# fabianschenk/REVO

Measured on AMD Instinct MI355X. Metric: tracked frames/sec at 640x480, 4-level pyramid; ATE vs reference, higher is better.
Workload: dtype f32

## Files before the change

include/revo_hip.h:

```cpp
#ifndef REVO_HIP_H
#define REVO_HIP_H

#include <stddef.h>
#include <stdint.h>

#ifdef __cplusplus
extern "C" {
#endif
#pragma GCC visibility push(default)

#define REVO_MAX_LEVELS 6

enum {
  REVO_OK = 0,
  REVO_ERR_INVALID_ARG = -1,
  REVO_ERR_HIP = -2,
  REVO_ERR_NOT_KEYFRAME = -3,
  REVO_ERR_NOT_ORTHOGONAL = -4,
  REVO_ERR_CAPACITY = -5,
  REVO_ERR_LEVEL = -6,
  REVO_ERR_UNSUPPORTED = -7,
  REVO_ERR_CORRUPT = -8
};

// ... 241 lines not shown
int revo_vo_keyframe(const revo_vo* v, revo_pyr** kf_out, float T_w_kf[16]);

typedef struct revo_vo_multi revo_vo_multi;
typedef struct revo_stream_frame {
  int32_t stream;
  const uint8_t* bgr; size_t bgr_stride;
  const void* depth; size_t depth_stride;
  double timestamp;
} revo_stream_frame;
typedef struct revo_stream_result {
  int32_t stream, new_keyframe;
  double timestamp;
  float pose[16];
} revo_stream_result;
int revo_vo_multi_create(revo_ctx* ctx, int n_streams, int max_queue, revo_vo_multi** out);
void revo_vo_multi_destroy(revo_vo_multi* m);
int revo_vo_multi_submit(revo_vo_multi* m, int n, const revo_stream_frame* frames,
                         int depth_is_u16, double depth_scale_factor);
int revo_vo_multi_step(revo_vo_multi* m, revo_stream_result* out, int* n_out);
int revo_vo_multi_pending(const revo_vo_multi* m, int stream);
int revo_vo_multi_reset(revo_vo_multi* m, int stream);
int revo_vo_multi_num_keyframes(const revo_vo_multi* m, int stream);
int revo_vo_multi_keyframe(const revo_vo_multi* m, int stream, revo_pyr** kf, float T_w_kf[16]);

int revo_vo_multi_submit_device(revo_vo_multi* m, int n, const revo_stream_frame* frames, int depth_is_u16,
                                double depth_scale_factor, void* producer_stream);

typedef struct revo_map revo_map;
int revo_map_create(revo_ctx* ctx, float voxel, int dense, size_t initial_voxels, size_t max_voxels, revo_map** out);
void revo_map_destroy(revo_map* m);
int revo_map_integrate(revo_map* m, const revo_pyr* kf, const float T_w_kf_colmajor[16]);
int revo_map_integrate_many(revo_map* m, int n, const revo_pyr* const* kfs, const float* T_w_kf_colmajor_n16);
int revo_map_clear(revo_map* m);
typedef struct revo_map_info_t {
  size_t voxels;
  size_t points_integrated;
  size_t points_dropped;
  size_t capacity;
  int32_t keyframes;
  int32_t keyframes_rejected;
  int32_t rehashes;
} revo_map_info_t;
int revo_map_info(revo_map* m, revo_map_info_t* out);
int revo_map_extract(revo_map* m, size_t min_count, float* xyz, uint8_t* rgb, uint32_t* count, size_t cap, size_t* n);
int revo_vo_multi_attach_map(revo_vo_multi* mv, int stream, revo_map* m);

typedef struct revo_map_view {
  int32_t width, height;
  float fx, fy, cx, cy, zmin, zmax;
  float T_w_c[16];
  int32_t splat_max;
  uint32_t min_count;
} revo_map_view;
int revo_map_render(revo_map* m, int n, const revo_map_view* views, float* const* depth, uint8_t* const* bgr, uint32_t* covered,
                    int device_out);
int revo_map_render_last_ms(revo_map* m, float* ms);

typedef struct revo_png_info {
  int32_t width, height, bit_depth, color_type, interlace;
  uint64_t idat_bytes;
  uint64_t raw_bytes;
} revo_png_info;
int revo_png_probe(const uint8_t* png, size_t len, revo_png_info* out);

enum { REVO_PNG_BGR8 = 0,
       REVO_PNG_U16 = 1    };
typedef struct revo_png_decoder revo_png_decoder;
int revo_png_decoder_create(revo_ctx* ctx, int max_images, size_t max_compressed_bytes, size_t max_raw_bytes_per_image,
                            revo_png_decoder** out);
void revo_png_decoder_destroy(revo_png_decoder* d);
typedef struct revo_png_job {
  const uint8_t* png; size_t len;
  int32_t format;
  int32_t width, height;
  void* d_dst; size_t dst_stride;
} revo_png_job;
int revo_png_decode_submit(revo_png_decoder* d, int n, const revo_png_job* jobs, void* stream, uint64_t* ticket);
int revo_png_decode_wait(revo_png_decoder* d, uint64_t ticket, int32_t* status);

int revo_debug_census_(int device, unsigned out3[3]);
int revo_debug_gate_timeouts_(int device);
void revo_debug_section_max_(unsigned long long out[12], int reset);
void revo_debug_wait_stats_(unsigned long long out[3]);
int revo_debug_track_profile_(revo_ctx* ctx, float out13[13]);
int revo_debug_batch_profile_(float* out, int n_pairs);

#pragma GCC visibility pop
#ifdef __cplusplus
}
#endif
#endif
```

revo_amd/csrc/revo_dev.h:

```cpp
#pragma once
#include <hip/hip_runtime.h>
#include <stdint.h>
#include "../../include/revo_hip.h"

#define REVO_L REVO_MAX_LEVELS

struct LevelGeom {
  int w, h;
  int npix;
  float fx, fy, cx, cy;
  int patch;
  int hist_w, hist_h;
  int nchunk;
  int chunk_rows;
  int wpr;
  int nms_block_base;
  int has_orig;
  int pix_base;
  int edt_rows;
  int edt_block_base;
  int strip_base;
  int cc_base;
  int band_rows, nbands, band_base;
};
// ... 19 lines not shown
struct FramePlanes {
  uint8_t* gray[REVO_L];
  float* depth[REVO_L];
  uint2* cs[REVO_L];
  uint8_t* edges[REVO_L];
  uint8_t* edges_orig[REVO_L];
  int* scratch[REVO_L];
  float4* pts[REVO_L];
  float4* pts_trk[REVO_L];
  float* dt[REVO_L];
  float4* table[REVO_L];
  uint8_t* hist[REVO_L];
  int* chunk[REVO_L];
  unsigned* cmask[REVO_L];
  uint8_t* vb[REVO_L];
  int* npts;
  int* hist_nz;
  int* strip_tot;
  uint32_t* ebits[REVO_L];
  int* need_full;
  int* hyst_heavy;
  int* tile_base;
  float* stage[REVO_L];
  unsigned short* epre[REVO_L];
  int* stage_base;
};

struct PairDesc {
  const float4* pts[REVO_L];
  const int* npts;
  const float* dt[REVO_L];
  float R[9];
  float T[3];
};

struct TrackParams {
  int pyr_min_lvl, pyr_max_lvl;
  int lvl_begin, lvl_end;
  int check_init;
  int eval_only;
  int kspec[REVO_L];
  int redundant_n;
  float lambda_success_fac, lambda_fail_fac;
  float lambda_initial[REVO_L], step_size_min[REVO_L], convergence_eps[REVO_L];
  int max_its[REVO_L];
  float edge_distance[REVO_L];
  float huber_edge;
  int use_edge_filter;
  struct { float fx, fy, cx, cy; int w, h; } cam[REVO_L];
  int exact_sums;
};

struct EvalOut {
  float A[36];
  float b[6];
  float error;
  float mean_err;
  float sum_w, sum_u;
  int good, bad;
};

#define REVO_MAX_WIDTH 2048
#define NMS_ROWS 6
#define EDT_ROW_PX 1280
#ifndef REVO_HYST_LDS_MAX
#define REVO_HYST_LDS_MAX 158720
#endif
#ifndef TRACK_THREADS
#define TRACK_THREADS 512
#endif
#ifndef TRACK_MAX_CLUSTER
#define TRACK_MAX_CLUSTER 32
#endif
#define TRACK_KMAX 4
#define TRACK_NVAL 48
#define TRACK_NVAL_X 132
#define TRACK_MAIL_NVAL TRACK_NVAL_X

void launch_gray_depth(const PyrGeom& g, const FramePlanes& p, const uint8_t* d_bgr, const float* d_depth_f32,
                       const uint16_t* d_depth_u16, float u16_alpha, int B, hipStream_t s);
void launch_pyrdown(const PyrGeom& g, const FramePlanes& p, int lvl, int B, hipStream_t s, int parts = 3, bool stage_edges = false);
void launch_edge_prefix(const PyrGeom& g, const FramePlanes& p, int B, hipStream_t s);
void launch_canny_nms(const PyrGeom& g, const FramePlanes& p, int B, hipStream_t s);
void launch_hyst(const PyrGeom& g, const FramePlanes& p, int B, hipStream_t s);
void launch_fill(const PyrGeom& g, const FramePlanes& p, int B, hipStream_t s);
void launch_compact(const PyrGeom& g, const FramePlanes& p, int B, hipStream_t s);
void launch_tile_points(const PyrGeom& g, const FramePlanes& p, int B, hipStream_t s, int which = 3);
void launch_pyrdown_bgr(const uint8_t* src, int w, int h, uint8_t* dst, hipStream_t s);
void launch_colored_pcl(const PyrGeom& g, const FramePlanes& p, int frame, int lvl, int dense, const uint8_t* bgr_lvl,
                        int* chunk, unsigned* cmask, int* total, int cap, float* out8, hipStream_t s);
void launch_keyframe(const PyrGeom& g, const FramePlanes& p, int f0, int fstride, int count, hipStream_t s, int which = 3);
int launch_track(const PairDesc* d_descs, const TrackParams& prm, revo_pair_result* d_out, EvalOut* d_eval,
                 int n_pairs, unsigned long long* d_mail, unsigned* epoch_io, int cluster, unsigned* d_resident, hipStream_t s);
void launch_track_gate(unsigned* d_resident, unsigned want, hipStream_t s);
int launch_track_one(const PairDesc& desc, const TrackParams& prm, revo_pair_result* out, EvalOut* eval_out,
                     unsigned long long* d_mail, unsigned* epoch_io, int cluster, unsigned* seq_ptr, unsigned seq_val,
                     unsigned* d_resident, hipStream_t s);
void launch_solve6(const float* d_Ab , int n, float* d_x , hipStream_t s);
int track_blocks_per_cu();
void launch_grad_table(const PyrGeom& g, const FramePlanes& p, int f0, int fstride, int count, hipStream_t s);
struct VoteArgs { float RT[3][12]; const float4* pts[3]; const int* n[3]; };
void launch_vote(const PyrGeom& g, const FramePlanes& curr, int curr_frame, int lvl, int n_clouds, const VoteArgs& va,
                 int* d_marks , int* d_hist8 , unsigned* d_done ,
                 int* h_out8 , unsigned seq_val, int use_orig_edges,
                 hipStream_t s);
void launch_copy_cloud(float4* dst, const float4* src, int* dst_n, const int* src_n, hipStream_t s);
struct VoteDesc {
  float RT[3][12]; const float4* pts[3]; const int* n[3]; int n_clouds;
  const uint8_t* edges; const float* depth;
  int* marks; int* hist8; unsigned* done;
  int* host_out;
};
struct CloudCopyDesc { float4* dst; const float4* src; int* dst_n; const int* src_n; };
struct CopySeg { const void* src; void* dst; size_t bytes; };
void launch_vote_multi(const PyrGeom& g, int lvl, int n, const VoteDesc* d_descs, unsigned seq_val, hipStream_t s);
void launch_copy_cloud_multi(int n, const CloudCopyDesc* d_descs, hipStream_t s);
void launch_copy_segments(int n, const CopySeg* d_segs, hipStream_t s);
```

revo_amd/csrc/revo_host.hip:

```cpp
#include <hip/hip_runtime.h>

#include <cmath>
#include <cstdio>
#include <chrono>
#include <cstring>
#include <atomic>
#include <deque>
#include <mutex>
#include <string>
#include <vector>

#include "revo_dev.h"
#include "revo_internal.h"
#include "revo_mat4.h"
#include "revo_multi.h"
#include "revo_map.h"

static thread_local std::string g_err;
extern "C" const char* revo_last_error(void) { return g_err.c_str(); }
extern "C" const char* revo_version(void) { return "0.1.0 gfx950"; }
extern "C" void revo_set_error_(const char* msg) { g_err = msg ? msg : ""; }

extern "C" void revo_pyr_settings_default(revo_pyr_settings* s) {
  memset(s, 0, sizeof(*s));
  s->width = 640; s->height = 480;
  s->fx = 517.306408f; s->fy = 516.469215f; s->cx = 318.643040f; s->cy = 255.313989f;
  s->pyr_min_lvl = 2; s->pyr_max_lvl = 0;
  s->canny_threshold1 = 150; s->canny_threshold2 = 100;
  s->depth_min = 0.1f; s->depth_max = 5.2f;
  s->use_edge_hist = 1; s->n_percentage = 0.3f;
  s->hist_patch[0] = 20; s->hist_patch[1] = 10; s->hist_patch[2] = 5;
}
extern "C" void revo_opt_settings_default(revo_opt_settings* s) {
  memset(s, 0, sizeof(*s));
  s->lambda_success_fac = 0.5f; s->lambda_fail_fac = 2.0f;
  const float ed[6] = {30, 20, 10, 5, 5, 5};
  for (int i = 0; i < REVO_L; ++i) {
    s->lambda_initial[i] = 0.f; s->step_size_min[i] = 1e-16f; s->convergence_eps[i] = 0.999f;
    s->max_its_per_lvl[i] = 100; s->edge_distance_lvl[i] = ed[i];
  }
  s->huber_edge = 0.3f;
  s->use_edge_filter = 1;
}
extern "C" void revo_tracker_settings_default(revo_tracker_settings* s) {
  s->check_tracking_results = 1; s->check_init_values = 1; s->n_frames_hist_voting = 3;
  s->histogram_level = 2;
}

struct FrameSet {
  int B = 0;
  void* blob = nullptr;
  size_t blob_bytes = 0;
  FramePlanes p{};
  float* own_depth0 = nullptr;
  uint8_t* d_bgr = nullptr;
  float* d_depth = nullptr;
  uint8_t* h_bgr = nullptr;
  float* h_depth = nullptr;
  hipEvent_t ev_ready = nullptr;
  hipStream_t ready_stream = nullptr;
  std::mutex edt_mu;
  std::atomic<bool> edt_pending{false};
  int edt_count = 0;
  hipEvent_t ev_edt = nullptr;
  hipStream_t edt_stream = nullptr;
  bool has_edt = false;
  std::atomic<bool> ref_lists_pending{false};
  hipEvent_t ev_ref = nullptr;
  hipStream_t ref_stream = nullptr;
  bool has_ref = false;
  hipEvent_t ev_free = nullptr;
  hipEvent_t ev_free2 = nullptr;
  hipEvent_t ev_h2d = nullptr;
  bool has_ready = false, has_free = false, has_free2 = false;
};

struct Past {
  float4* d_pts; int* d_n; int n; float T_w[16]; double ts;
  size_t cap;
};

struct Knobs {
  int track_depth;
  int cluster_one;
  int redundant_one;
  int direct_h2d;
  int h2d_max_run_mb;
  bool kspec_one_set;
  int kspec_one[REVO_L];
  int upload_blocks;
  int h2d_kernel;
  int stage_edge_depths;
};

struct revo_ctx {
  std::atomic<int> refs{1};
  int device;
  Knobs knobs;
  revo_pyr_settings ps; revo_opt_settings os; revo_tracker_settings ts;
  PyrGeom geom;
  TrackParams tp;
  hipStream_t stream;
  hipStream_t build_stream;
  std::mutex mu;
  std::vector<FrameSet*> pool;
  int framesets_created = 0;
  std::vector<Past> past_pool;
  PairDesc* h_desc;
  revo_pair_result* h_res;
  EvalOut* h_eval;
  unsigned* h_seq;
  unsigned seq_next = 1;
  unsigned long long* d_mail;
  unsigned mail_epoch = 0;
  int num_cus, blocks_per_cu;
  std::deque<Past> past;
  int* d_marks; int* d_hist8; int* h_hist8; unsigned* d_vote_done;
  std::vector<struct revo_pairs_job*> jobs;
  hipStream_t copy_stream = nullptr, copy_stream2 = nullptr, pair_streams[2] = {nullptr, nullptr};
  hipStream_t vote_stream = nullptr;
  hipEvent_t ev_vote = nullptr;
  hipStream_t frame_copy_stream = nullptr;
  unsigned long long jobs_submitted = 0;
  char* d_pcl = nullptr; float* d_pcl_out; uint8_t* d_pcl_clr[2]; int* d_pcl_chunk; unsigned* d_pcl_mask; int* d_pcl_total;
};

struct revo_pyr {
  revo_ctx* ctx;
  FrameSet* fs;
  int frame;
  bool owns_fs;
  bool is_kf;
  double ts;
  bool table_built;
  bool ref_list_built;
  bool dt_ready = false;
  bool has_colour = false;
};

struct revo_batch {
  revo_ctx* ctx;
  int n_pairs;
  FrameSet* fs;
  std::vector<revo_pyr> views;
  PairDesc* h_descs; PairDesc* d_descs;
  unsigned long long* d_mail;
  unsigned mail_epoch = 0;
  bool identity_uploaded = false;
  int cluster;
  bool defer = true;
  hipStream_t stream;
  hipEvent_t ev0, ev1, ev_upload;
  hipEvent_t ev_trk = nullptr;
// ... 170 lines not shown
  return REVO_OK;
}
extern "C" int revo_debug_gate_timeouts_(int device) {
  TrackChain& ch = g_chain[device & 63];
  std::lock_guard<std::mutex> lk(ch.mu);
  if (!ch.d_resident) return -1;
  unsigned v = 0;
  if (hipMemcpy(&v, ch.d_resident + 1, sizeof(unsigned), hipMemcpyDeviceToHost) != hipSuccess) return -2;
  return (int)v;
}
extern "C" int revo_debug_census_(int device, unsigned out3[3]) {
  TrackChain& ch = g_chain[device & 63];
  std::lock_guard<std::mutex> lk(ch.mu);
  if (!ch.d_resident || !out3) return -1;
  if (hipMemcpy(out3, ch.d_resident, 2 * sizeof(unsigned), hipMemcpyDeviceToHost) != hipSuccess) return -2;
  out3[2] = ch.started_total;
  return 0;
}
static size_t mail_bytes(int n_pairs, int cluster) { return sizeof(unsigned long long) * (size_t)n_pairs * 2 * cluster * TRACK_MAIL_NVAL; }

static size_t align_up(size_t v, size_t a) { return (v + a - 1) / a * a; }

static int frameset_create(revo_ctx* c, int B, bool with_staging, FrameSet** out, bool host_staging = true) {
  const PyrGeom& g = c->geom;
  FrameSet* fs = new FrameSet();
  fs->B = B;
  for (int pass = 0; pass < 2; ++pass) {
    size_t off = 0;
    auto take = [&](size_t bytes) -> void* {
      void* p = pass ? (void*)((char*)fs->blob + off) : nullptr;
      off = align_up(off + bytes, 256);
      return p;
    };
    for (int l = 0; l < g.n_levels; ++l) {
      const LevelGeom& v = g.lv[l];
      const size_t n = (size_t)v.npix * B;
      fs->p.gray[l] = (uint8_t*)take(n);
      fs->p.depth[l] = (float*)take(n * 4);
      fs->p.cs[l] = (uint2*)take((size_t)v.h * v.wpr * 8 * B);
      fs->p.edges[l] = (uint8_t*)take(n);
      fs->p.edges_orig[l] = (uint8_t*)take(n);
      fs->p.scratch[l] = (int*)take(n * 4);
      fs->p.pts[l] = (float4*)take(n * 16);
      fs->p.pts_trk[l] = (float4*)take(n * 16);
      fs->p.dt[l] = (float*)take(n * 4);
      fs->p.table[l] = (float4*)take(n * 16);
      fs->p.hist[l] = (uint8_t*)take((size_t)std::max(1, v.hist_w * v.hist_h) * B);
      fs->p.chunk[l] = (int*)take((size_t)v.w * v.nchunk * B * 4);
      fs->p.cmask[l] = (unsigned*)take((size_t)v.w * v.nchunk * B * 4);
      fs->p.vb[l] = (uint8_t*)take((n + 7) / 8);
      fs->p.ebits[l] = (uint32_t*)take((size_t)v.h * v.wpr * 4 * B);
      if (B > 1 && l < g.n_levels - 1) {
        fs->p.stage[l] = (float*)take(n * 4);
        fs->p.epre[l] = (unsigned short*)take((size_t)v.h * v.wpr * 2 * B);
      }
    }
    fs->own_depth0 = fs->p.depth[0];
    fs->p.npts = (int*)take(sizeof(int) * REVO_L * B);
    fs->p.hist_nz = (int*)take(sizeof(int) * REVO_L * B);
    fs->p.strip_tot = (int*)take(sizeof(int) * (size_t)g.total_strips * B);
    fs->p.tile_base = (int*)take(sizeof(int) * (size_t)g.total_tiles * B);
    fs->p.need_full = (int*)take(sizeof(int) * REVO_L * B);
    fs->p.hyst_heavy = (int*)take(sizeof(int) * B);
    fs->p.stage_base = (int*)take(sizeof(int) * (size_t)g.total_tiles * B);
    if (with_staging) {
      fs->d_bgr = (uint8_t*)take((size_t)g.lv[0].npix * 3 * B);
      fs->d_depth = (float*)take((size_t)g.lv[0].npix * 4 * B);
    }
    if (!pass) {
      fs->blob_bytes = off;
      hipError_t e = hipMalloc(&fs->blob, off);
      if (e != hipSuccess) { delete fs; return fail(REVO_ERR_HIP, std::string("hipMalloc: ") + hipGetErrorString(e)); }
    }
  }
  if (with_staging && host_staging) {
    HIPCHECK(hipHostMalloc((void**)&fs->h_bgr, (size_t)g.lv[0].npix * 3 * B));
    HIPCHECK(hipHostMalloc((void**)&fs->h_depth, (size_t)g.lv[0].npix * 4 * B));
  }
  HIPCHECK(hipEventCreateWithFlags(&fs->ev_ready, hipEventDisableTiming));
  HIPCHECK(hipEventCreateWithFlags(&fs->ev_free, hipEventDisableTiming));
  HIPCHECK(hipEventCreateWithFlags(&fs->ev_free2, hipEventDisableTiming));
  HIPCHECK(hipEventCreateWithFlags(&fs->ev_edt, hipEventDisableTiming));
  HIPCHECK(hipEventCreateWithFlags(&fs->ev_ref, hipEventDisableTiming));
  hipMemsetAsync(fs->p.npts, 0, sizeof(int) * REVO_L * B, c->stream);
  HIPCHECK(hipStreamSynchronize(c->stream));
  *out = fs;
  return REVO_OK;
}
static void frameset_destroy(FrameSet* fs) {
  if (!fs) return;
  if (fs->blob) hipFree(fs->blob);
  if (fs->h_bgr) hipHostFree(fs->h_bgr);
  if (fs->h_depth) hipHostFree(fs->h_depth);
  if (fs->ev_ready) hipEventDestroy(fs->ev_ready);
  if (fs->ev_free) hipEventDestroy(fs->ev_free);
  if (fs->ev_free2) hipEventDestroy(fs->ev_free2);
  if (fs->ev_edt) hipEventDestroy(fs->ev_edt);
  if (fs->ev_ref) hipEventDestroy(fs->ev_ref);
  if (fs->ev_h2d) hipEventDestroy(fs->ev_h2d);
  delete fs;
}

static void enqueue_build(revo_ctx* c, FrameSet* fs, const uint8_t* d_bgr, const float* d_depth_f32,
                          const uint16_t* d_depth_u16, float alpha, hipStream_t s, bool borrow_depth = false,
                          bool with_points = true, int frame0 = 0, int nframes = -1, bool gray_only = false) {
  PyrGeom g = c->geom;
  g.frame0 = frame0;
  const int B = nframes < 0 ? fs->B : nframes;
  fs->p.depth[0] = (borrow_depth && d_depth_f32) ? const_cast<float*>(d_depth_f32) : fs->own_depth0;
  launch_gray_depth(g, fs->p, d_bgr, d_depth_f32, d_depth_u16, alpha, B, s);
  for (int l = 1; l < g.n_levels; ++l) launch_pyrdown(g, fs->p, l, B, s, gray_only ? 1 : 3);
  launch_canny_nms(g, fs->p, B, s);
  launch_hyst(g, fs->p, B, s);
  launch_fill(g, fs->p, B, s);
  if (with_points) launch_tile_points(g, fs->p, B, s);
}

static int enqueue_batch_tail(revo_batch* b, hipStream_t s);
static int batch_wait_tracker(revo_batch* b, hipStream_t s);

static void ctx_free(revo_ctx* c);
extern "C" int revo_ctx_create(int device, const revo_pyr_settings* pyr, const revo_opt_settings* opt,
                               const revo_tracker_settings* trk, revo_ctx** out) {
  if (!pyr || !out) return fail(REVO_ERR_INVALID_ARG, "null argument");
  int ndev = 0;
  if (hipGetDeviceCount(&ndev) != hipSuccess || ndev <= 0)
    return fail(REVO_ERR_HIP, "no HIP device: librevo_hip has no CPU fallback");
  if (device < 0 || device >= ndev) return fail(REVO_ERR_INVALID_ARG, "device ordinal out of range");
  HIPCHECK(hipSetDevice(device));
  revo_ctx* c = new revo_ctx();
  c->device = device;
  c->ps = *pyr;
  c->knobs.track_depth = env_track_depth();
  c->knobs.cluster_one = env_int("REVO_TRACK_CLUSTER_ONE", 0, 0, TRACK_MAX_CLUSTER);
  c->knobs.redundant_one = env_int("REVO_TRACK_REDUNDANT_ONE", 1024, 0, 1 << 30);
  c->knobs.direct_h2d = env_int("REVO_DIRECT_H2D", 1, 0, 1);
  c->knobs.stage_edge_depths = env_int("REVO_STAGE_EDGE_DEPTHS", 0, 0, 1);
  {
    const char* e1 = getenv("REVO_TRACK_KSPEC_ONE");
    const char* eb = getenv("REVO_TRACK_KSPEC");
    const size_t n1 = e1 ? strlen(e1) : 0;
    c->knobs.kspec_one_set = n1 > 0 || !(eb && *eb);
    for (int i = 0; i < REVO_L; ++i) {
      int k = i < 2 ? 3 : TRACK_KMAX;
      if (n1 == 1) k = e1[0] - '0'; else if (n1 > 1) k = e1[std::min<size_t>(i, n1 - 1)] - '0';
      c->knobs.kspec_one[i] = std::max(1, std::min(TRACK_KMAX, k));
    }
  }
  c->knobs.upload_blocks = env_int("REVO_UPLOAD_BLOCKS", 64, 1, 4096);
  c->knobs.h2d_kernel = env_int("REVO_H2D_KERNEL", 0, 0, 1);
  c->knobs.h2d_max_run_mb = env_int("REVO_H2D_MAX_RUN_MB", 64, 1, 4096);
  if (opt) c->os = *opt; else revo_opt_settings_default(&c->os);
  if (trk) c->ts = *trk; else revo_tracker_settings_default(&c->ts);
  std::string why;
  if (build_geom(c->ps, &c->geom, &why)) { delete c; return fail(REVO_ERR_INVALID_ARG, why); }
  build_track_params(c, &c->tp);
  struct Guard { revo_ctx* c; ~Guard() { if (c) ctx_free(c); } } guard{c};
  HIPCHECK(hipStreamCreateWithFlags(&c->stream, hipStreamNonBlocking));
  HIPCHECK(hipStreamCreateWithFlags(&c->build_stream, hipStreamNonBlocking));
  HIPCHECK(hipStreamCreateWithFlags(&c->vote_stream, hipStreamNonBlocking));
  HIPCHECK(hipEventCreateWithFlags(&c->ev_vote, hipEventDisableTiming));
  HIPCHECK(hipHostMalloc((void**)&c->h_desc, sizeof(PairDesc)));
  HIPCHECK(hipHostMalloc((void**)&c->h_res, sizeof(revo_pair_result) * 3));
  HIPCHECK(hipHostMalloc((void**)&c->h_seq, sizeof(unsigned) * 4));
  memset(c->h_seq, 0, sizeof(unsigned) * 4);
  HIPCHECK(hipHostMalloc((void**)&c->h_eval, sizeof(EvalOut)));
  hipDeviceProp_t prop;
  HIPCHECK(hipGetDeviceProperties(&prop, device));
  c->num_cus = prop.multiProcessorCount;
  c->blocks_per_cu = std::min(track_blocks_per_cu(), 2);
  HIPCHECK(hipMalloc((void**)&c->d_mail, mail_bytes(1, TRACK_MAX_CLUSTER)));
  HIPCHECK(hipMemset(c->d_mail, 0, mail_bytes(1, TRACK_MAX_CLUSTER)));
  size_t maxpix = 0;
  for (int l = 0; l < c->geom.n_levels; ++l) maxpix = std::max(maxpix, (size_t)c->geom.lv[l].npix);
  HIPCHECK(hipMalloc((void**)&c->d_marks, sizeof(int) * maxpix));
  HIPCHECK(hipMalloc((void**)&c->d_hist8, sizeof(int) * 8));
  HIPCHECK(hipMalloc((void**)&c->d_vote_done, sizeof(unsigned)));
  HIPCHECK(hipMemset(c->d_marks, 0, sizeof(int) * maxpix));
  HIPCHECK(hipMemset(c->d_hist8, 0, sizeof(int) * 8));
  HIPCHECK(hipMemset(c->d_vote_done, 0, sizeof(unsigned)));
  HIPCHECK(hipHostMalloc((void**)&c->h_hist8, sizeof(int) * 16));
  memset(c->h_hist8, 0, sizeof(int) * 16);
  HIPCHECK(hipDeviceSynchronize());
  guard.c = nullptr;
  *out = c;
  return REVO_OK;
}

static void ctx_free(revo_ctx* c) {
  hipSetDevice(c->device);
  if (c->build_stream) hipStreamSynchronize(c->build_stream);
  if (c->stream) hipStreamSynchronize(c->stream);
  if (c->vote_stream) { (void)hipStreamSynchronize(c->vote_stream); (void)hipStreamDestroy(c->vote_stream); }
  if (c->ev_vote) (void)hipEventDestroy(c->ev_vote);
  for (int k = 0; k < 2; ++k) if (c->pair_streams[k]) (void)hipStreamDestroy(c->pair_streams[k]);
  if (c->copy_stream) (void)hipStreamDestroy(c->copy_stream);
  if (c->copy_stream2) (void)hipStreamDestroy(c->copy_stream2);
// ... 26 lines not shown
      if (c->framesets_created >= total) return REVO_OK;
      c->framesets_created += 1;
    }
    FrameSet* fs = nullptr;
    const int rc = frameset_create(c, 1, true, &fs);
    std::lock_guard<std::mutex> lk(c->mu);
    if (rc) { c->framesets_created -= 1; return rc; }
    c->pool.push_back(fs);
  }
}
extern "C" int revo_ctx_device_(const revo_ctx* c) { return c ? c->device : -1; }
extern "C" void revo_ctx_retain_(revo_ctx* c) { if (c) ctx_ref(c); }
extern "C" void revo_ctx_release_(revo_ctx* c) { if (c) ctx_unref(c); }

extern "C" int revo_ctx_set_tracker(revo_ctx* c, const revo_opt_settings* opt, const revo_tracker_settings* trk) {
  if (!c) return fail(REVO_ERR_INVALID_ARG, "null context");
  std::lock_guard<std::mutex> lk(c->mu);
  if (opt) c->os = *opt;
  if (trk) c->ts = *trk;
  const int exact = c->tp.exact_sums;
  build_track_params(c, &c->tp);
  c->tp.exact_sums = exact;
  while (!c->past.empty()) { c->past_pool.push_back(c->past.front()); c->past.pop_front(); }
  return REVO_OK;
}

extern "C" int revo_ctx_histogram_level(const revo_ctx* c) { return c ? c->ts.histogram_level : -1; }

extern "C" int revo_ctx_set_exact_sums(revo_ctx* c, int on) {
  if (!c) return fail(REVO_ERR_INVALID_ARG, "null context");
  std::lock_guard<std::mutex> lk(c->mu);
  c->tp.exact_sums = on ? 1 : 0;
  return REVO_OK;
}
extern "C" int revo_ctx_exact_sums(const revo_ctx* c) { return c ? c->tp.exact_sums : -1; }

extern "C" int revo_ctx_camera(const revo_ctx* c, int lvl, float out6[6]) {
  if (!c || !out6) return fail(REVO_ERR_INVALID_ARG, "null argument");
  if (lvl < 0 || lvl >= c->geom.n_levels) return fail(REVO_ERR_LEVEL, "level out of range");
  const LevelGeom& v = c->geom.lv[lvl];
  out6[0] = v.fx; out6[1] = v.fy; out6[2] = v.cx; out6[3] = v.cy; out6[4] = (float)v.w; out6[5] = (float)v.h;
  return REVO_OK;
}

static void enqueue_list_side(revo_ctx* c, FrameSet* fs, int f0, int fstride, int count, hipStream_t s) {
  PyrGeom gp = c->geom;
  gp.frame0 = f0; gp.fstride = fstride;
  const bool stage = c->knobs.stage_edge_depths && fs->p.stage[0] != nullptr && c->geom.n_levels > 1;
  if (stage) launch_edge_prefix(gp, fs->p, count, s);
  for (int l = 1; l < c->geom.n_levels; ++l) launch_pyrdown(gp, fs->p, l, count, s, 2, stage);
  gp.pts_staged = stage ? 1 : 0;
  launch_tile_points(gp, fs->p, count, s);
}
static int run_pending_edt(revo_ctx* c, FrameSet* fs, hipStream_t s, bool need_ref_lists = false) {
  std::lock_guard<std::mutex> lk(fs->edt_mu);
  bool behind_build = false;
  if (!fs->edt_pending) {
    if (fs->has_edt && fs->edt_stream != s) HIPCHECK(hipStreamWaitEvent(s, fs->ev_edt, 0));
  } else {
    if (fs->has_ready) HIPCHECK(hipStreamWaitEvent(s, fs->ev_ready, 0));
    behind_build = true;
    enqueue_list_side(c, fs, 1, 2, fs->edt_count, s);
    launch_keyframe(c->geom, fs->p, 0, 2, fs->edt_count, s);
    HIPCHECK(hipGetLastError());
    HIPCHECK(hipEventRecord(fs->ev_edt, s));
    fs->has_edt = true;
    fs->edt_stream = s;
    fs->edt_pending = false;
  }
  if (!need_ref_lists) return REVO_OK;
  if (!fs->ref_lists_pending) {
    if (fs->has_ref && fs->ref_stream != s) HIPCHECK(hipStreamWaitEvent(s, fs->ev_ref, 0));
    return REVO_OK;
  }
  if (!behind_build && fs->has_ready) HIPCHECK(hipStreamWaitEvent(s, fs->ev_ready, 0));
  enqueue_list_side(c, fs, 0, 2, fs->edt_count, s);
  HIPCHECK(hipGetLastError());
  HIPCHECK(hipEventRecord(fs->ev_ref, s));
  fs->has_ref = true;
  fs->ref_stream = s;
  fs->ref_lists_pending = false;
  return REVO_OK;
}
static int wait_edt_before_rebuild(FrameSet* fs, hipStream_t s) {
  std::lock_guard<std::mutex> lk(fs->edt_mu);
  if (fs->has_edt && fs->edt_stream != s) HIPCHECK(hipStreamWaitEvent(s, fs->ev_edt, 0));
  if (fs->has_ref && fs->ref_stream != s) HIPCHECK(hipStreamWaitEvent(s, fs->ev_ref, 0));
  return REVO_OK;
}
typedef unsigned v4u __attribute__((ext_vector_type(4)));
__global__ void __launch_bounds__(256) k_upload_rows(uint8_t* __restrict__ dst, const uint8_t* __restrict__ src, size_t src_stride,
                                                     size_t row_bytes, int rows) {
  const size_t vec = row_bytes / 16, tail0 = vec * 16;
  for (int y = blockIdx.y; y < rows; y += gridDim.y) {
    const uint8_t* s = src + (size_t)y * src_stride;
    uint8_t* d = dst + (size_t)y * row_bytes;
    const bool aligned = (((uintptr_t)s | (uintptr_t)d) & 15) == 0;
    if (aligned) {
      for (size_t i = blockIdx.x * blockDim.x + threadIdx.x; i < vec; i += (size_t)gridDim.x * blockDim.x)
        ((v4u*)d)[i] = __builtin_nontemporal_load((const v4u*)s + i);
      for (size_t i = tail0 + blockIdx.x * blockDim.x + threadIdx.x; i < row_bytes; i += (size_t)gridDim.x * blockDim.x) d[i] = s[i];
    } else {
      for (size_t i = blockIdx.x * blockDim.x + threadIdx.x; i < row_bytes; i += (size_t)gridDim.x * blockDim.x) d[i] = s[i];
    }
  }
}
static hipError_t upload_rows(void* dst, const void* src, size_t src_stride, size_t row_bytes, int rows, int max_blocks, hipStream_t s) {
  void* dsrc = nullptr;
  hipError_t e = hipHostGetDevicePointer(&dsrc, const_cast<void*>(src), 0);
  if (e != hipSuccess) { (void)hipGetLastError(); return e; }
  if (src_stride == row_bytes) {
    const size_t bytes = row_bytes * rows;
    const int blocks = (int)std::min<size_t>((size_t)max_blocks, (bytes / 16 + 255) / 256 + 1);
    hipLaunchKernelGGL(k_upload_rows, dim3(blocks, 1), dim3(256), 0, s, (uint8_t*)dst, (const uint8_t*)dsrc, bytes, bytes, 1);
  } else {
    hipLaunchKernelGGL(k_upload_rows, dim3(2, std::min(rows, 128)), dim3(256), 0, s, (uint8_t*)dst, (const uint8_t*)dsrc, src_stride, row_bytes, rows);
  }
  return hipGetLastError();
}
static std::atomic<unsigned long long> g_sec_max_ns[12];
extern "C" void revo_debug_section_max_(unsigned long long out[12], int reset) {
  for (int i = 0; i < 12; ++i) { out[i] = g_sec_max_ns[i].load(); if (reset) g_sec_max_ns[i].store(0); }
}
extern "C" void revo_debug_section_note_(int i, unsigned long long ns) {
  if (i < 0 || i >= 12) return;
  unsigned long long cur = g_sec_max_ns[i].load(std::memory_order_relaxed);
  while (ns > cur && !g_sec_max_ns[i].compare_exchange_weak(cur, ns)) {}
}
struct SecTimer {
  std::chrono::steady_clock::time_point t = std::chrono::steady_clock::now();
  void lap(int i) {
    const auto n = std::chrono::steady_clock::now();
    revo_debug_section_note_(i, (unsigned long long)std::chrono::duration_cast<std::chrono::nanoseconds>(n - t).count());
    t = n;
  }
};
static int wait_event_polled(hipEvent_t ev) {
  const auto t0 = std::chrono::steady_clock::now();
  for (unsigned spin = 0;; ++spin) {
    const hipError_t e = hipEventQuery(ev);
    if (e == hipSuccess) return REVO_OK;
    if (e != hipErrorNotReady) { (void)hipGetLastError(); return fail(REVO_ERR_HIP, std::string("hipEventQuery: ") + hipGetErrorString(e)); }
    (void)hipGetLastError();
    for (int k = 0; k < 32; ++k) __builtin_ia32_pause();
    if ((spin & 1023) == 1023 && std::chrono::steady_clock::now() - t0 > std::chrono::seconds(2)) break;
  }
  HIPCHECK(hipEventSynchronize(ev));
  return REVO_OK;
}
static int wait_ready_on(revo_ctx* c, const revo_pyr* p, hipStream_t s) {
  if (p->fs->has_ready) HIPCHECK(hipStreamWaitEvent(s, p->fs->ev_ready, 0));
  return run_pending_edt(c, p->fs, s, (p->frame & 1) == 0);
}
static int wait_ready(revo_ctx* c, const revo_pyr* p) { return wait_ready_on(c, p, c->stream); }
static int vote_enqueued(revo_ctx* c, const revo_pyr* p) {
  if (p->owns_fs) return REVO_OK;
  HIPCHECK(hipEventRecord(c->ev_vote, c->vote_stream));
  HIPCHECK(hipStreamWaitEvent(c->stream, c->ev_vote, 0));
  return REVO_OK;
}

static int pyramid_create_common(revo_ctx* c, const uint8_t* bgr, size_t bgr_stride, const void* depth,
                                 size_t depth_stride, bool is_u16, double scale, double ts, revo_pyr** out) {
  if (!c || !bgr || !depth || !out) return fail(REVO_ERR_INVALID_ARG, "null argument");
  HIPCHECK(hipSetDevice(c->device));
  const int w = c->geom.lv[0].w, h = c->geom.lv[0].h;
  if (bgr_stride < (size_t)w * 3 || depth_stride < (size_t)w * (is_u16 ? 2 : 4))
    return fail(REVO_ERR_INVALID_ARG, "stride smaller than a row");
  FrameSet* fs = nullptr;
  SecTimer sec;
  {
    std::lock_guard<std::mutex> lk(c->mu);
    if (!c->pool.empty()) { fs = c->pool.back(); c->pool.pop_back(); }
  }
  sec.lap(0);
  if (!fs) {
    int rc = frameset_create(c, 1, true, &fs);
    if (rc) return rc;
    std::lock_guard<std::mutex> lk(c->mu);
    c->framesets_created += 1;
  }
  const size_t brow = (size_t)w * 3, drow = (size_t)w * (is_u16 ? 2 : 4);
  hipStream_t bs = c->build_stream;
  auto page_locked = [](const void* p) {
    hipPointerAttribute_t at;
    if (hipPointerGetAttributes(&at, p) != hipSuccess) { (void)hipGetLastError(); return false; }
    return at.type == hipMemoryTypeHost;
  };
  const bool direct = c->knobs.direct_h2d && page_locked(bgr) && page_locked(depth) &&
                      page_locked(bgr + (size_t)(h - 1) * bgr_stride + brow - 1) &&
                      page_locked((const char*)depth + (size_t)(h - 1) * depth_stride + drow - 1);
  sec.lap(1);
  if (direct) {
    {
      std::lock_guard<std::mutex> lk(c->mu);
      if (!c->frame_copy_stream) HIPCHECK(hipStreamCreateWithFlags(&c->frame_copy_stream, hipStreamNonBlocking));
    }
    if (!fs->ev_h2d) HIPCHECK(hipEventCreateWithFlags(&fs->ev_h2d, hipEventDisableTiming));
    hipStream_t cs = c->frame_copy_stream;
    if (fs->has_ready) HIPCHECK(hipStreamWaitEvent(cs, fs->ev_ready, 0));
    if (fs->has_free) HIPCHECK(hipStreamWaitEvent(cs, fs->ev_free, 0));
    if (fs->has_free2) HIPCHECK(hipStreamWaitEvent(cs, fs->ev_free2, 0));
    sec.lap(6);
    if (c->knobs.h2d_kernel && upload_rows(fs->d_bgr, bgr, bgr_stride, brow, h, c->knobs.upload_blocks, cs) == hipSuccess) {}
    else if (bgr_stride == brow) HIPCHECK(hipMemcpyAsync(fs->d_bgr, bgr, brow * h, hipMemcpyHostToDevice, cs));
    else HIPCHECK(hipMemcpy2DAsync(fs->d_bgr, brow, bgr, bgr_stride, brow, h, hipMemcpyHostToDevice, cs));
    sec.lap(7);
    if (c->knobs.h2d_kernel && upload_rows(fs->d_depth, depth, depth_stride, drow, h, c->knobs.upload_blocks, cs) == hipSuccess) {}
    else if (depth_stride == drow) HIPCHECK(hipMemcpyAsync(fs->d_depth, depth, drow * h, hipMemcpyHostToDevice, cs));
    else HIPCHECK(hipMemcpy2DAsync(fs->d_depth, drow, depth, depth_stride, drow, h, hipMemcpyHostToDevice, cs));
    sec.lap(8);
    HIPCHECK(hipEventRecord(fs->ev_h2d, cs));
    sec.lap(9);
    HIPCHECK(hipStreamWaitEvent(bs, fs->ev_h2d, 0));
    sec.lap(2);
    { int rc = wait_event_polled(fs->ev_h2d); if (rc) return rc; }
    sec.lap(3);
  } else {
    if (fs->has_ready) HIPCHECK(hipEventSynchronize(fs->ev_ready));
    for (int y = 0; y < h; ++y) memcpy(fs->h_bgr + (size_t)y * brow, bgr + (size_t)y * bgr_stride, brow);
    for (int y = 0; y < h; ++y) memcpy((char*)fs->h_depth + (size_t)y * drow, (const char*)depth + (size_t)y * depth_stride, drow);
    if (fs->has_free) HIPCHECK(hipStreamWaitEvent(bs, fs->ev_free, 0));
    if (fs->has_free2) HIPCHECK(hipStreamWaitEvent(bs, fs->ev_free2, 0));
    HIPCHECK(hipMemcpyAsync(fs->d_bgr, fs->h_bgr, brow * h, hipMemcpyHostToDevice, bs));
    HIPCHECK(hipMemcpyAsync(fs->d_depth, fs->h_depth, drow * h, hipMemcpyHostToDevice, bs));
  }
  const float alpha = is_u16 ? (float)(1.0f / scale) : 0.0f;
  enqueue_build(c, fs, fs->d_bgr, is_u16 ? nullptr : fs->d_depth, is_u16 ? (const uint16_t*)fs->d_depth : nullptr, alpha, bs, true);
  HIPCHECK(hipGetLastError());
  HIPCHECK(hipEventRecord(fs->ev_ready, bs));
  sec.lap(4);
  fs->has_ready = true;
  fs->ready_stream = bs;
  revo_pyr* p = new revo_pyr{c, fs, 0, true, false, ts, false, false};
  ctx_ref(c);
  *out = p;
  return REVO_OK;
}

extern "C" int revo_pyramid_create(revo_ctx* ctx, const uint8_t* bgr, size_t bgr_stride, const float* depth_m,
                                   size_t depth_stride, double timestamp, revo_pyr** out) {
  return pyramid_create_common(ctx, bgr, bgr_stride, depth_m, depth_stride, false, 1.0, timestamp, out);
}
extern "C" int revo_pyramid_create_u16(revo_ctx* ctx, const uint8_t* bgr, size_t bgr_stride, const uint16_t* depth_raw,
                                       size_t depth_stride, double depth_scale_factor, double timestamp, revo_pyr** out) {
  if (!(depth_scale_factor > 0)) return fail(REVO_ERR_INVALID_ARG, "depth_scale_factor must be > 0");
  return pyramid_create_common(ctx, bgr, bgr_stride, depth_raw, depth_stride, true, depth_scale_factor, timestamp, out);
}

extern "C" void revo_pyramid_destroy(revo_pyr* p) {
  if (!p) return;
  if (p->owns_fs) {
    hipSetDevice(p->ctx->device);
    std::lock_guard<std::mutex> lk(p->ctx->mu);
    hipEventRecord(p->fs->ev_free, p->ctx->stream);
    p->fs->has_free = true;
    hipEventRecord(p->fs->ev_free2, p->ctx->vote_stream);
    p->fs->has_free2 = true;
    p->ctx->pool.push_back(p->fs);
  }
  revo_ctx* c = p->owns_fs ? p->ctx : nullptr;
  delete p;
  if (c) ctx_unref(c);
}

extern "C" int revo_pyramid_make_keyframe(revo_pyr* p) {
  if (!p) return fail(REVO_ERR_INVALID_ARG, "null pyramid");
  HIPCHECK(hipSetDevice(p->ctx->device));
  { int rc = wait_ready(p->ctx, p); if (rc) return rc; }
  if (!p->dt_ready) launch_keyframe(p->ctx->geom, p->fs->p, p->frame, 1, 1, p->ctx->stream);
  HIPCHECK(hipGetLastError());
  p->dt_ready = false;
  p->is_kf = true;
  p->table_built = false;
  return REVO_OK;
}
extern "C" int revo_pyramid_prepare_keyframe_(revo_pyr* p) {
  if (!p) return fail(REVO_ERR_INVALID_ARG, "null pyramid");
  if (!p->owns_fs || p->is_kf || p->dt_ready) return REVO_OK;
  HIPCHECK(hipSetDevice(p->ctx->device));
  { int rc = wait_ready(p->ctx, p); if (rc) return rc; }
  launch_keyframe(p->ctx->geom, p->fs->p, p->frame, 1, 1, p->ctx->stream);
  HIPCHECK(hipGetLastError());
  p->dt_ready = true;
  return REVO_OK;
}
extern "C" int revo_pyramid_is_keyframe(const revo_pyr* p) { return p && p->is_kf; }
extern "C" double revo_pyramid_timestamp(const revo_pyr* p) { return p ? p->ts : 0.0; }

extern "C" int revo_pyramid_read(revo_pyr* p, revo_plane what, int lvl, void* dst, size_t cap, size_t* count) {
  if (!p) return fail(REVO_ERR_INVALID_ARG, "null pyramid");
  revo_ctx* c = p->ctx;
  HIPCHECK(hipSetDevice(c->device));
  if (lvl < 0 || lvl >= c->geom.n_levels) return fail(REVO_ERR_LEVEL, "level out of range");
  const LevelGeom& v = c->geom.lv[lvl];
  const FramePlanes& P = p->fs->p;
  const size_t f = (size_t)p->frame;
  { int rc = wait_ready(c, p); if (rc) return rc; }
  HIPCHECK(hipStreamSynchronize(c->stream));
  const void* src = nullptr;
  size_t n = v.npix, esz = 1;
  switch (what) {
    case REVO_PLANE_GRAY: src = P.gray[lvl] + f * v.npix; break;
    case REVO_PLANE_DEPTH: src = P.depth[lvl] + f * v.npix; esz = 4; break;
    case REVO_PLANE_EDGES: src = P.edges[lvl] + f * v.npix; break;
    case REVO_PLANE_EDGES_ORIG:
      src = (v.has_orig ? P.edges_orig[lvl] : P.edges[lvl]) + f * v.npix;
      break;
    case REVO_PLANE_DT:
      if (!p->is_kf) return fail(REVO_ERR_NOT_KEYFRAME, "distance transform not built: call makeKeyframe");
      src = P.dt[lvl] + f * v.npix; esz = 4; break;
    case REVO_PLANE_GRADTABLE:
      if (!p->is_kf) return fail(REVO_ERR_NOT_KEYFRAME, "optimizationStructure not built");
      if (!p->table_built) {
        launch_grad_table(c->geom, P, p->frame, 1, 1, c->stream);
        HIPCHECK(hipGetLastError());
        HIPCHECK(hipStreamSynchronize(c->stream));
        p->table_built = true;
      }
      src = P.table[lvl] + f * v.npix; esz = 16; break;
    case REVO_PLANE_EDGES3D: {
      if (!p->ref_list_built) {
        PyrGeom g1 = c->geom;
        g1.frame0 = p->frame;
        launch_compact(g1, P, 1, c->stream);
        HIPCHECK(hipGetLastError());
        HIPCHECK(hipStreamSynchronize(c->stream));
        p->ref_list_built = true;
      }
      int np = 0;
      HIPCHECK(hipMemcpy(&np, P.npts + f * REVO_L + lvl, sizeof(int), hipMemcpyDeviceToHost));
      n = (size_t)np; src = P.pts[lvl] + f * v.npix; esz = 16; break;
    }
    case REVO_PLANE_EDGES3D_TILED: {
      int np = 0;
      HIPCHECK(hipMemcpy(&np, P.npts + f * REVO_L + lvl, sizeof(int), hipMemcpyDeviceToHost));
      n = (size_t)np; src = P.pts_trk[lvl] + f * v.npix; esz = 16; break;
    }
    case REVO_PLANE_HIST:
      if (v.patch <= 0) { n = 0; src = P.hist[lvl]; break; }
      n = (size_t)v.hist_w * v.hist_h; src = P.hist[lvl] + f * n; break;
    default: return fail(REVO_ERR_INVALID_ARG, "unknown plane");
  }
  if (count) *count = n;
  if (dst) {
    if (n * esz > cap) return fail(REVO_ERR_CAPACITY, "host buffer too small");
    if (n) HIPCHECK(hipMemcpy(dst, src, n * esz, hipMemcpyDeviceToHost));
  }
  return REVO_OK;
}

extern "C" int revo_pyramid_colored_pcl(revo_pyr* p, int lvl, int dense, float* dst8, size_t cap_points, size_t* count) {
  if (!p) return fail(REVO_ERR_INVALID_ARG, "null pyramid");
  revo_ctx* c = p->ctx;
  HIPCHECK(hipSetDevice(c->device));
  if (lvl < 0 || lvl >= c->geom.n_levels) return fail(REVO_ERR_LEVEL, "level out of range");
  if (!(p->owns_fs || p->has_colour) || !p->fs->d_bgr)
    return fail(REVO_ERR_INVALID_ARG, "batch views keep no colour image (rgbFullSize): use revo_pyramid_create");
  { int rc = wait_ready(c, p); if (rc) return rc; }
  std::lock_guard<std::mutex> lk(c->mu);
  const PyrGeom& g = c->geom;
  const size_t n0 = g.lv[0].npix, slots = (size_t)g.lv[0].w * g.lv[0].nchunk;
  if (!c->d_pcl) {
    size_t off = 0;
    auto take = [&](size_t bytes) { size_t o = off; off += (bytes + 255) & ~(size_t)255; return o; };
    const size_t o_out = take(n0 * 32), o_a = take(n0 / 4 * 3 + 3), o_b = take(n0 / 16 * 3 + 3), o_ch = take(slots * 4),
                 o_m = take(slots * 4), o_t = take(4);
    HIPCHECK(hipMalloc((void**)&c->d_pcl, off));
    c->d_pcl_out = (float*)(c->d_pcl + o_out);
    c->d_pcl_clr[0] = (uint8_t*)(c->d_pcl + o_a); c->d_pcl_clr[1] = (uint8_t*)(c->d_pcl + o_b);
    c->d_pcl_chunk = (int*)(c->d_pcl + o_ch); c->d_pcl_mask = (unsigned*)(c->d_pcl + o_m); c->d_pcl_total = (int*)(c->d_pcl + o_t);
  }
  hipStream_t s = c->stream;
  const uint8_t* clr = p->fs->d_bgr + (size_t)p->frame * n0 * 3;
  for (int l = 0; l < lvl; ++l) {
    uint8_t* d = c->d_pcl_clr[l & 1];
    launch_pyrdown_bgr(clr, g.lv[l].w, g.lv[l].h, d, s);
    clr = d;
  }
  const int cap = (int)std::min<size_t>(dst8 ? cap_points : 0, (size_t)g.lv[lvl].npix);
  launch_colored_pcl(g, p->fs->p, p->frame, lvl, dense ? 1 : 0, clr, c->d_pcl_chunk, c->d_pcl_mask, c->d_pcl_total,
                     dst8 ? cap : g.lv[lvl].npix, c->d_pcl_out, s);
  HIPCHECK(hipGetLastError());
  int total = 0;
  HIPCHECK(hipMemcpyAsync(&total, c->d_pcl_total, sizeof(int), hipMemcpyDeviceToHost, s));
  HIPCHECK(hipStreamSynchronize(s));
  if (count) *count = (size_t)total;
  if (dst8) {
    if ((size_t)total > cap_points) return fail(REVO_ERR_CAPACITY, "host buffer too small");
    if (total) HIPCHECK(hipMemcpy(dst8, c->d_pcl_out, (size_t)total * 32, hipMemcpyDeviceToHost));
  }
  return REVO_OK;
}

extern "C" int revo_map_source_(revo_pyr* p, MapSource* out) {
  if (!p || !out) return fail(REVO_ERR_INVALID_ARG, "null pyramid");
  revo_ctx* c = p->ctx;
  HIPCHECK(hipSetDevice(c->device));
  if (!(p->owns_fs || p->has_colour) || !p->fs->d_bgr)
    return fail(REVO_ERR_INVALID_ARG, "batch views keep no colour image (rgbFullSize): use revo_pyramid_create");
  { int rc = wait_ready(c, p); if (rc) return rc; }
  const size_t n0 = c->geom.lv[0].npix, f = (size_t)p->frame;
  out->ctx = c;
  out->depth = p->fs->p.depth[0] + f * n0;
  out->edges = p->fs->p.edges[0] + f * n0;
  out->bgr = p->fs->d_bgr + f * n0 * 3;
  return REVO_OK;
}
extern "C" int revo_map_ctx_geom_(const revo_ctx* c, MapCtxGeom* out) {
  if (!c || !out) return fail(REVO_ERR_INVALID_ARG, "null context");
  const LevelGeom& l = c->geom.lv[0];
  *out = MapCtxGeom{c->device, l.w, l.h, l.fx, l.fy, l.cx, l.cy, c->geom.depth_min, c->geom.depth_max, (void*)c->stream};
  return REVO_OK;
}

static void fill_desc(PairDesc* d, const revo_pyr* ref, const revo_pyr* curr, const float* R, const float* T) {
  const PyrGeom& g = ref->ctx->geom;
  memset(d, 0, sizeof(*d));
  for (int l = 0; l < g.n_levels; ++l) {
    d->pts[l] = curr->fs->p.pts_trk[l] + (size_t)curr->frame * g.lv[l].npix;
    d->dt[l] = ref->fs->p.dt[l] + (size_t)ref->frame * g.lv[l].npix;
  }
  d->npts = curr->fs->p.npts + (size_t)curr->frame * REVO_L;
  if (R) memcpy(d->R, R, sizeof(float) * 9); else { d->R[0] = d->R[4] = d->R[8] = 1.f; }
  if (T) memcpy(d->T, T, sizeof(float) * 3);
}

static int check_pair(const revo_ctx* c, const revo_pyr* ref, const revo_pyr* curr) {
  if (!c || !ref || !curr) return fail(REVO_ERR_INVALID_ARG, "null argument");
  if (ref->ctx != c || curr->ctx != c) return fail(REVO_ERR_INVALID_ARG, "pyramid belongs to another context");
  if (!ref->is_kf) return fail(REVO_ERR_NOT_KEYFRAME, "optimizationStructure not built! (reference frame is not a keyframe)");
  return REVO_OK;
}

static std::atomic<unsigned long long> g_wait_fallbacks{0}, g_wait_max_ns{0}, g_wait_calls{0};
extern "C" void revo_debug_wait_stats_(unsigned long long out[3]) {
  out[0] = g_wait_calls.load(); out[1] = g_wait_fallbacks.load(); out[2] = g_wait_max_ns.load();
}
static int wait_seq(hipStream_t s, volatile unsigned* word, unsigned want) {
  static const int spin_limit = env_int("REVO_WAIT_SPINS", 200000, 1000, 2000000000);
  const auto t0 = std::chrono::steady_clock::now();
  g_wait_calls.fetch_add(1, std::memory_order_relaxed);
  auto note = [&]() {
    const unsigned long long ns = (unsigned long long)std::chrono::duration_cast<std::chrono::nanoseconds>(std::chrono::steady_clock::now() - t0).count();
    unsigned long long cur = g_wait_max_ns.load(std::memory_order_relaxed);
    while (ns > cur && !g_wait_max_ns.compare_exchange_weak(cur, ns)) {}
  };
  for (int spin = 0; spin < spin_limit; ++spin) {
    if (*word == want) { std::atomic_thread_fence(std::memory_order_acquire); note(); return REVO_OK; }
    __builtin_ia32_pause();
  }
  g_wait_fallbacks.fetch_add(1, std::memory_order_relaxed);
  HIPCHECK(hipStreamSynchronize(s));
  note();
  if (*word != want) return fail(REVO_ERR_HIP, "a kernel finished without publishing its result");
  return REVO_OK;
}

static int track_launch(revo_ctx* c, const revo_pyr* ref, const revo_pyr* curr, const float* R, const float* T,
                        const TrackParams& tp, int slot, unsigned* seq_out) {
  fill_desc(c->h_desc, ref, curr, R, T);
  { int rc = wait_ready(c, ref); if (rc) return rc; rc = wait_ready(c, curr); if (rc) return rc; }
  TrackParams tp1 = tp;
  tp1.redundant_n = c->knobs.redundant_one;
  if (c->knobs.kspec_one_set)
    for (int i = 0; i < REVO_L; ++i) tp1.kspec[i] = c->knobs.kspec_one[i];
  const unsigned seq = c->seq_next++;
  if (c->seq_next == 0) c->seq_next = 1;
  const int rc = chained_track_launch(c->device, c->knobs.track_depth, c->stream, [&](unsigned* d_resident) {
    return launch_track_one(*c->h_desc, tp1, c->h_res + slot, c->h_eval, c->d_mail, &c->mail_epoch, pick_cluster(c, 1), c->h_seq + slot,
                            seq, d_resident, c->stream);
  });
  if (rc) return rc;
  *seq_out = seq;
  return REVO_OK;
}
static int track_wait(revo_ctx* c, int slot, unsigned seq) { return wait_seq(c->stream, c->h_seq + slot, seq); }

enum { SINGLE_SLOT = 2 };
static int run_single(revo_ctx* c, const revo_pyr* ref, const revo_pyr* curr, const float* R, const float* T,
                      const TrackParams& tp) {
  unsigned seq = 0;
  int rc = track_launch(c, ref, curr, R, T, tp, SINGLE_SLOT, &seq);
  if (rc) return rc;
// ... 31 lines not shown
  int rc = track_wait(c, slot & 1, seq);
  if (rc) return rc;
  return decode_track(c->h_res[slot & 1], R, T, err, status, nullptr, nullptr);
}

extern "C" int revo_optimizer_track_level(revo_ctx* c, const revo_pyr* ref, const revo_pyr* curr, float R[9], float T[3],
                                          int lvl, revo_residual_info* info, float* err) {
  int rc = check_pair(c, ref, curr);
  if (rc) return rc;
  if (!R || !T) return fail(REVO_ERR_INVALID_ARG, "null pose");
  if (lvl < 0 || lvl >= c->geom.n_levels) return fail(REVO_ERR_LEVEL, "level out of range");
  HIPCHECK(hipSetDevice(c->device));
  std::lock_guard<std::mutex> lk(c->mu);
  TrackParams tp = c->tp;
  tp.lvl_begin = tp.lvl_end = lvl; tp.check_init = 0; tp.eval_only = 0;
  rc = run_single(c, ref, curr, R, T, tp);
  if (rc) return rc;
  return decode_track(c->h_res[SINGLE_SLOT], R, T, err, nullptr, info, nullptr);
}

extern "C" int revo_optimizer_eval(revo_ctx* c, const revo_pyr* ref, const revo_pyr* curr, const float R[9],
                                   const float T[3], int lvl, revo_residual_info* info, float* err, float A[36],
                                   float b[6]) {
  int rc = check_pair(c, ref, curr);
  if (rc) return rc;
  if (!R || !T) return fail(REVO_ERR_INVALID_ARG, "null pose");
  if (lvl < 0 || lvl >= c->geom.n_levels) return fail(REVO_ERR_LEVEL, "level out of range");
  HIPCHECK(hipSetDevice(c->device));
  std::lock_guard<std::mutex> lk(c->mu);
  TrackParams tp = c->tp;
  tp.lvl_begin = tp.lvl_end = lvl; tp.check_init = 0; tp.eval_only = 1;
  rc = run_single(c, ref, curr, R, T, tp);
  if (rc) return rc;
  const EvalOut& e = *c->h_eval;
  if (info) { info->good_pts_edges = e.good; info->bad_pts_edges = e.bad; info->sum_error_unweighted = e.sum_u; info->sum_error_weighted = e.sum_w; }
  if (err) *err = e.mean_err;
  if (A) memcpy(A, e.A, sizeof(float) * 36);
  if (b) memcpy(b, e.b, sizeof(float) * 6);
  return REVO_OK;
}

extern "C" int revo_optimizer_solve6(revo_ctx* c, int n, const float* A36_b6_lambda, float* x6) {
  if (!c || !A36_b6_lambda || !x6 || n <= 0) return fail(REVO_ERR_INVALID_ARG, "bad argument");
  HIPCHECK(hipSetDevice(c->device));
  std::lock_guard<std::mutex> lk(c->mu);
  float *d_in = nullptr, *d_out = nullptr;
  HIPCHECK(hipMalloc((void**)&d_in, sizeof(float) * 43 * (size_t)n));
  hipError_t e = hipMalloc((void**)&d_out, sizeof(float) * 6 * (size_t)n);
  if (e == hipSuccess) e = hipMemcpyAsync(d_in, A36_b6_lambda, sizeof(float) * 43 * (size_t)n, hipMemcpyHostToDevice, c->stream);
  if (e == hipSuccess) { launch_solve6(d_in, n, d_out, c->stream); e = hipGetLastError(); }
  if (e == hipSuccess) e = hipMemcpyAsync(x6, d_out, sizeof(float) * 6 * (size_t)n, hipMemcpyDeviceToHost, c->stream);
  if (e == hipSuccess) e = hipStreamSynchronize(c->stream);
  hipFree(d_in); hipFree(d_out);
  if (e != hipSuccess) return fail(REVO_ERR_HIP, std::string("revo_optimizer_solve6: ") + hipGetErrorString(e));
  return REVO_OK;
}

extern "C" int revo_debug_track_profile_(revo_ctx* c, float out13[13]) {
  if (!c || !out13) return REVO_ERR_INVALID_ARG;
  memcpy(out13, c->h_eval->A, sizeof(float) * 13);
  return REVO_OK;
}

extern "C" int revo_tracker_track_frames(revo_ctx* c, const revo_pyr* ref, const revo_pyr* curr, float R[9], float T[3],
                                         float* err, int* status, revo_residual_info* info, int32_t iters[REVO_MAX_LEVELS]) {
  int rc = check_pair(c, ref, curr);
  if (rc) return rc;
  if (!R || !T) return fail(REVO_ERR_INVALID_ARG, "null pose");
  HIPCHECK(hipSetDevice(c->device));
  std::lock_guard<std::mutex> lk(c->mu);
  TrackParams tp = c->tp;
  tp.eval_only = 0;
  rc = run_single(c, ref, curr, R, T, tp);
  if (rc) return rc;
  return decode_track(c->h_res[SINGLE_SLOT], R, T, err, status, info, iters);
}

static int assess_launch(revo_ctx* c, const float T_w_curr[16], const revo_pyr* curr, int* nframes_out, unsigned* seq_out) {
  *nframes_out = -1;
  if (c->past.empty() || !c->ts.check_tracking_results) return REVO_OK;
  const int hl = c->ts.histogram_level;
  if (hl < 0 || hl >= c->geom.n_levels) return fail(REVO_ERR_LEVEL, "histogram_level outside the pyramid");
  hipStream_t vs = c->vote_stream;
  { int rc = wait_ready_on(c, curr, vs); if (rc) return rc; }
  float inv[16];
  mat4_inverse(T_w_curr, inv);
  int nframes = 0;
  VoteArgs va{};
  for (int fr = 0; fr < c->ts.n_frames_hist_voting && fr < (int)c->past.size() && fr < 3; ++fr) {
    float tf[16];
    mat4_mul(inv, c->past[fr].T_w, tf);
    float* RT = va.RT[fr];
    for (int cc = 0; cc < 3; ++cc) for (int r = 0; r < 3; ++r) RT[cc * 3 + r] = tf[cc * 4 + r];
    RT[9] = tf[12]; RT[10] = tf[13]; RT[11] = tf[14];
    va.pts[fr] = c->past[fr].d_pts;
    va.n[fr] = c->past[fr].d_n;
    ++nframes;
  }
  const int use_orig = c->geom.lv[hl].has_orig;
  const unsigned seq = c->seq_next++;
  if (c->seq_next == 0) c->seq_next = 1;
  launch_vote(c->geom, curr->fs->p, curr->frame, hl, nframes, va, c->d_marks, c->d_hist8, c->d_vote_done, c->h_hist8, seq,
              use_orig, vs);
  HIPCHECK(hipGetLastError());
  { int rc = vote_enqueued(c, curr); if (rc) return rc; }
  *nframes_out = nframes;
  *seq_out = seq;
  return REVO_OK;
}
static int assess_wait(revo_ctx* c, int nframes, unsigned seq, int* status, int32_t hist4[4], int32_t overlaps4[4]) {
  if (status) *status = REVO_TRACKER_STATE_OK;
  if (nframes < 0) return REVO_OK;
  hipStream_t vs = c->vote_stream;
  { int rc = wait_seq(vs, (volatile unsigned*)(c->h_hist8 + 8), seq); if (rc) return rc; }
  const int* hist = c->h_hist8;
  const int* ov = c->h_hist8 + 4;
  const float wts[4] = {0.f, 1.f, 1.25f, 1.5f};
  float overlapMeasure = 0.0f;
  const int hsize = 1 + nframes;
  for (int k = 1; k < hsize; ++k) overlapMeasure += (ov[k] * wts[k]);
  if (hist4) memcpy(hist4, hist, sizeof(int32_t) * 4);
  if (overlaps4) memcpy(overlaps4, ov, sizeof(int32_t) * 4);
  if (status) *status = (overlapMeasure >= ov[0] || hsize < 4) ? REVO_TRACKER_STATE_OK : REVO_TRACKER_STATE_NEW_KF;
  return REVO_OK;
}

extern "C" int revo_tracker_assess_quality(revo_ctx* c, const float T_w_curr[16], const revo_pyr* curr, int* status,
                                           int32_t hist4[4], int32_t overlaps4[4]) {
  if (!c || !T_w_curr || !curr) return fail(REVO_ERR_INVALID_ARG, "null argument");
  if (curr->ctx != c) return fail(REVO_ERR_INVALID_ARG, "pyramid belongs to another context");
  if (hist4) memset(hist4, 0, sizeof(int32_t) * 4);
  if (overlaps4) memset(overlaps4, 0, sizeof(int32_t) * 4);
  if (status) *status = REVO_TRACKER_STATE_OK;
  HIPCHECK(hipSetDevice(c->device));
  std::lock_guard<std::mutex> lk(c->mu);
  int nframes = -1;
  unsigned seq = 0;
  int rc = assess_launch(c, T_w_curr, curr, &nframes, &seq);
  if (rc) return rc;
  return assess_wait(c, nframes, seq, status, hist4, overlaps4);
}
extern "C" int revo_assess_launch_(revo_ctx* c, const float T_w_curr[16], const revo_pyr* curr, int* nframes_out, unsigned* seq_out) {
  if (!c || !T_w_curr || !curr || curr->ctx != c) return fail(REVO_ERR_INVALID_ARG, "bad argument");
  HIPCHECK(hipSetDevice(c->device));
  std::lock_guard<std::mutex> lk(c->mu);
  return assess_launch(c, T_w_curr, curr, nframes_out, seq_out);
}
extern "C" int revo_assess_wait_(revo_ctx* c, int nframes, unsigned seq, int* status, float* ratio_out) {
  if (!c) return fail(REVO_ERR_INVALID_ARG, "null context");
  int32_t ov[4] = {0, 0, 0, 0};
  const int rc = assess_wait(c, nframes, seq, status, nullptr, ov);
  if (ratio_out) {
    *ratio_out = INFINITY;
    if (rc == REVO_OK && nframes >= 3 && ov[0] > 0) {
      const float wts[4] = {0.f, 1.f, 1.25f, 1.5f};
      float m = 0.0f;
      for (int k = 1; k < 1 + nframes && k < 4; ++k) m += ov[k] * wts[k];
      *ratio_out = m / (float)ov[0];
    }
  }
  return rc;
}

static int past_take(revo_ctx* c, size_t need, Past* out) {
  for (size_t k = 0; k < c->past_pool.size(); ++k)
    if (c->past_pool[k].cap >= need) { *out = c->past_pool[k]; c->past_pool.erase(c->past_pool.begin() + k); return REVO_OK; }
  Past p{};
// ... 51 lines not shown
  std::lock_guard<std::mutex> lk(c->mu);
  while ((int)c->past.size() > c->ts.n_frames_hist_voting) {
    c->past_pool.push_back(c->past.front());
    c->past.pop_front();
  }
  return REVO_OK;
}
extern "C" void revo_tracker_reset_past_(revo_ctx* c) {
  if (!c) return;
  std::lock_guard<std::mutex> lk(c->mu);
  while (!c->past.empty()) { c->past_pool.push_back(c->past.front()); c->past.pop_front(); }
}
extern "C" int revo_tracker_past_size(const revo_ctx* c) { return c ? (int)c->past.size() : 0; }

static bool env_defer() {
  return env_int("REVO_EDT_DEFER", 1, 0, 1) && env_int("REVO_DEFER", 2, 0, 3) != 0;
}
extern "C" int revo_batch_create(revo_ctx* c, int n_pairs, revo_batch** out) {
  if (!c || !out || n_pairs <= 0) return fail(REVO_ERR_INVALID_ARG, "bad argument");
  HIPCHECK(hipSetDevice(c->device));
  revo_batch* b = new revo_batch();
  b->ctx = c; b->n_pairs = n_pairs;
  ctx_ref(c);
  int rc = frameset_create(c, 2 * n_pairs, false, &b->fs);
  if (rc) { delete b; ctx_unref(c); return rc; }
  struct Guard { revo_batch* b; ~Guard() { if (b) revo_batch_destroy(b); } } guard{b};
  HIPCHECK(hipStreamCreateWithFlags(&b->stream, hipStreamNonBlocking));
  HIPCHECK(hipEventCreate(&b->ev0)); HIPCHECK(hipEventCreate(&b->ev1));
  HIPCHECK(hipEventCreateWithFlags(&b->ev_upload, hipEventDisableTiming));
  HIPCHECK(hipEventCreateWithFlags(&b->ev_trk, hipEventDisableTiming));
  b->cluster = pick_cluster(c, n_pairs);
  b->defer = env_defer();
  HIPCHECK(hipMalloc((void**)&b->d_mail, mail_bytes(n_pairs, b->cluster)));
  HIPCHECK(hipMemset(b->d_mail, 0, mail_bytes(n_pairs, b->cluster)));
  for (int f = 0; f < 2 * n_pairs; ++f) b->views.push_back(revo_pyr{c, b->fs, f, false, (f % 2) == 0, 0.0, false, false});
  HIPCHECK(hipHostMalloc((void**)&b->h_descs, sizeof(PairDesc) * n_pairs));
  HIPCHECK(hipHostMalloc((void**)&b->h_flags, sizeof(revo_pair_result) * n_pairs));
  HIPCHECK(hipMalloc((void**)&b->d_descs, sizeof(PairDesc) * n_pairs));
  for (int i = 0; i < n_pairs; ++i) fill_desc(&b->h_descs[i], &b->views[2 * i], &b->views[2 * i + 1], nullptr, nullptr);
  HIPCHECK(hipStreamSynchronize(c->stream));
  HIPCHECK(hipStreamSynchronize(nullptr));
  guard.b = nullptr;
  *out = b;
  return REVO_OK;
}
extern "C" void revo_batch_destroy(revo_batch* b) {
  if (!b) return;
  hipSetDevice(b->ctx->device);
  if (b->stream) hipStreamSynchronize(b->stream);
  hipHostFree(b->h_descs); hipHostFree(b->h_flags); hipFree(b->d_descs); hipFree(b->d_mail);
  if (b->ev0) hipEventDestroy(b->ev0);
  if (b->ev1) hipEventDestroy(b->ev1);
  if (b->ev_upload) hipEventDestroy(b->ev_upload);
  if (b->ev_trk) hipEventDestroy(b->ev_trk);
  if (b->stream) hipStreamDestroy(b->stream);
  frameset_destroy(b->fs);
  revo_ctx* c = b->ctx;
  delete b;
  ctx_unref(c);
}

static int batch_wait_tracker(revo_batch* b, hipStream_t s) {
  if (b->has_trk && b->trk_stream != s) HIPCHECK(hipStreamWaitEvent(s, b->ev_trk, 0));
  return REVO_OK;
}
static int batch_wait_build(revo_batch* b, hipStream_t s) {
  if (b->defer) return REVO_OK;
  if (b->fs->has_ready && b->fs->ready_stream != s) HIPCHECK(hipStreamWaitEvent(s, b->fs->ev_ready, 0));
  return REVO_OK;
}
static int batch_mark_tracker(revo_batch* b, hipStream_t s) {
  HIPCHECK(hipEventRecord(b->ev_trk, s));
  b->has_trk = true;
  b->trk_stream = s;
  return REVO_OK;
}

static int enqueue_batch_tail(revo_batch* b, hipStream_t s) {
  const PyrGeom& g = b->ctx->geom;
  if (b->defer) {
    std::lock_guard<std::mutex> lk(b->fs->edt_mu);
    b->fs->edt_pending = true; b->fs->edt_count = b->n_pairs;
    b->fs->ref_lists_pending = true;
  } else {
    launch_tile_points(g, b->fs->p, b->fs->B, s);
    launch_keyframe(g, b->fs->p, 0, 2, b->n_pairs, s);
  }
  return REVO_OK;
}

static int batch_build_f32(revo_batch* b, const uint8_t* d_bgr, const float* d_depth, void* stream, bool borrow) {
  if (!b || !d_bgr || !d_depth) return fail(REVO_ERR_INVALID_ARG, "null argument");
  HIPCHECK(hipSetDevice(b->ctx->device));
  hipStream_t s = stream ? (hipStream_t)stream : b->stream;
  { int rc = wait_edt_before_rebuild(b->fs, s); if (rc) return rc; }
  { int rc = batch_wait_tracker(b, s); if (rc) return rc; }
  enqueue_build(b->ctx, b->fs, d_bgr, d_depth, nullptr, 0.f, s, borrow, false, 0, -1, b->defer);
  { int rc = enqueue_batch_tail(b, s); if (rc) return rc; }
  HIPCHECK(hipGetLastError());
  HIPCHECK(hipEventRecord(b->fs->ev_ready, s));
  b->fs->has_ready = true;
  b->fs->ready_stream = s;
  for (auto& v : b->views) { v.table_built = false; v.ref_list_built = false; }
  return REVO_OK;
}
extern "C" int revo_batch_build(revo_batch* b, const uint8_t* d_bgr, const float* d_depth, void* stream) {
  return batch_build_f32(b, d_bgr, d_depth, stream, false);
}
extern "C" int revo_batch_build_borrow(revo_batch* b, const uint8_t* d_bgr, const float* d_depth, void* stream) {
  return batch_build_f32(b, d_bgr, d_depth, stream, true);
}

static int batch_upload_init(revo_batch* b, const float* h_init_RT, hipStream_t s) {
  if (!h_init_RT && b->identity_uploaded) return REVO_OK;
  b->identity_uploaded = (h_init_RT == nullptr);
  HIPCHECK(hipEventSynchronize(b->ev_upload));
  for (int i = 0; i < b->n_pairs; ++i) {
    PairDesc& d = b->h_descs[i];
    if (h_init_RT) { memcpy(d.R, h_init_RT + 12 * i, sizeof(float) * 9); memcpy(d.T, h_init_RT + 12 * i + 9, sizeof(float) * 3); }
    else { memset(d.R, 0, sizeof(d.R)); d.R[0] = d.R[4] = d.R[8] = 1.f; memset(d.T, 0, sizeof(d.T)); }
  }
  HIPCHECK(hipMemcpyAsync(b->d_descs, b->h_descs, sizeof(PairDesc) * b->n_pairs, hipMemcpyHostToDevice, s));
  HIPCHECK(hipEventRecord(b->ev_upload, s));
  return REVO_OK;
}

extern "C" int revo_batch_prepare(revo_batch* b, void* stream) {
  if (!b) return fail(REVO_ERR_INVALID_ARG, "null argument");
  HIPCHECK(hipSetDevice(b->ctx->device));
  hipStream_t s = stream ? (hipStream_t)stream : b->stream;
  return run_pending_edt(b->ctx, b->fs, s);
}

extern "C" int revo_batch_track_only(revo_batch* b, const float* h_init_RT, revo_pair_result* d_results, void* stream) {
  if (!b || !d_results) return fail(REVO_ERR_INVALID_ARG, "null argument");
  HIPCHECK(hipSetDevice(b->ctx->device));
  hipStream_t s = stream ? (hipStream_t)stream : b->stream;
  { int rc0 = batch_wait_tracker(b, s); if (rc0) return rc0; }
  int rc = batch_upload_init(b, h_init_RT, s);
  if (rc) return rc;
  TrackParams tp = b->ctx->tp;
  tp.eval_only = 0;
  { int rc1 = batch_wait_build(b, s); if (rc1) return rc1; }
  { int rc2 = run_pending_edt(b->ctx, b->fs, s); if (rc2) return rc2; }
  b->last_results = d_results;
  rc = chained_track_launch(b->ctx->device, b->ctx->knobs.track_depth, s, [&](unsigned* d_resident) {
    if (b->tev0) (void)hipEventRecord(b->tev0, s);
    const int n_wg = launch_track(b->d_descs, tp, d_results, nullptr, b->n_pairs, b->d_mail, &b->mail_epoch, b->cluster, d_resident, s);
    if (b->tev1) (void)hipEventRecord(b->tev1, s);
    b->tev0 = b->tev1 = nullptr;
    return n_wg;
  });
  if (rc) return rc;
  return batch_mark_tracker(b, s);
}
extern "C" void revo_batch_time_next_grid_(revo_batch* b, void* ev0, void* ev1) {
  if (b) { b->tev0 = (hipEvent_t)ev0; b->tev1 = (hipEvent_t)ev1; }
}

extern "C" int revo_batch_build_u16(revo_batch* b, const uint8_t* d_bgr, const uint16_t* d_depth_raw,
                                    double depth_scale_factor, void* stream) {
  if (!b || !d_bgr || !d_depth_raw) return fail(REVO_ERR_INVALID_ARG, "null argument");
  if (!(depth_scale_factor > 0.0)) return fail(REVO_ERR_INVALID_ARG, "depth_scale_factor must be positive");
  HIPCHECK(hipSetDevice(b->ctx->device));
  hipStream_t s = stream ? (hipStream_t)stream : b->stream;
  { int rc = wait_edt_before_rebuild(b->fs, s); if (rc) return rc; }
// ... 212 lines not shown
extern "C" int revo_track_pairs(revo_ctx* c, int n, const revo_pair_in* pairs, int depth_is_u16, double depth_scale_factor,
                                revo_pair_out* out) {
  revo_pairs_job* j = nullptr;
  const int rc = revo_track_pairs_submit(c, n, pairs, depth_is_u16, depth_scale_factor, &j);
  if (rc) return rc;
  return revo_track_pairs_wait(j, out);
}

extern "C" int revo_batch_profile_build(revo_batch* b, const uint8_t* d_bgr, const float* d_depth, int reps, revo_stage_times* out) {
  if (!b || !d_bgr || !d_depth || !out || reps <= 0) return fail(REVO_ERR_INVALID_ARG, "bad argument");
  revo_ctx* c = b->ctx;
  HIPCHECK(hipSetDevice(c->device));
  hipStream_t s = b->stream;
  { int rc = wait_edt_before_rebuild(b->fs, s); if (rc) return rc; }
  { int rc = batch_wait_tracker(b, s); if (rc) return rc; }
  memset(out, 0, sizeof(*out));
  PyrGeom g = c->geom;
  g.frame0 = 0;
  FrameSet* fs = b->fs;
  const int B = fs->B, L = g.n_levels;
  fs->p.depth[0] = const_cast<float*>(d_depth);
  struct Stage { const char* name; int a, w; };
  std::vector<Stage> st;
  st.push_back({"k_gray_depth", 0, 0});
  for (int l = 1; l < L; ++l) st.push_back({"k_pyrdown_gray", l, 1});
  st.push_back({"k_canny_nms4", 0, 0});
  st.push_back({"hysteresis", 0, 0});
  st.push_back({"k_fill", 0, 0});
  const bool stage = c->knobs.stage_edge_depths && fs->p.stage[0] != nullptr && L > 1;
  PyrGeom gp = g;
  gp.pts_staged = stage ? 1 : 0;
  if (stage) st.push_back({"k_edge_prefix", 0, 0});
  for (int l = 1; l < L; ++l) st.push_back({"k_pyrdown_depth", l, 2});
  st.push_back({"k_tile_count", 0, 1});
  st.push_back({"k_pts_tiles", 0, 2});
  st.push_back({"k_edt_cols", 0, 1});
  st.push_back({"k_edt_rows", 0, 2});
  const int n = (int)st.size();
  if (n > REVO_MAX_STAGES) return fail(REVO_ERR_CAPACITY, "too many stages");
  struct Events {
    std::vector<hipEvent_t> v;
    ~Events() { for (hipEvent_t e : v) if (e) (void)hipEventDestroy(e); }
  } evs;
  evs.v.assign(n + 1, nullptr);
  std::vector<hipEvent_t>& ev = evs.v;
  for (auto& e : ev) HIPCHECK(hipEventCreate(&e));
  std::vector<double> sum(n, 0.0);
  for (int r = 0; r < reps; ++r) {
    HIPCHECK(hipEventRecord(ev[0], s));
    for (int i = 0; i < n; ++i) {
      const std::string nm = st[i].name;
      if (nm == "k_gray_depth") launch_gray_depth(g, fs->p, d_bgr, d_depth, nullptr, 0.f, B, s);
      else if (nm == "k_pyrdown_gray") launch_pyrdown(g, fs->p, st[i].a, B, s, 1);
      else if (nm == "k_pyrdown_depth") launch_pyrdown(g, fs->p, st[i].a, B, s, 2, stage);
      else if (nm == "k_edge_prefix") launch_edge_prefix(g, fs->p, B, s);
      else if (nm == "k_canny_nms4") launch_canny_nms(g, fs->p, B, s);
      else if (nm == "hysteresis") launch_hyst(g, fs->p, B, s);
      else if (nm == "k_fill") launch_fill(g, fs->p, B, s);
      else if (nm == "k_tile_count" || nm == "k_pts_tiles") launch_tile_points(gp, fs->p, B, s, st[i].w);
      else launch_keyframe(g, fs->p, 0, 2, b->n_pairs, s, st[i].w);
      HIPCHECK(hipGetLastError());
      HIPCHECK(hipEventRecord(ev[i + 1], s));
    }
    HIPCHECK(hipStreamSynchronize(s));
    for (int i = 0; i < n; ++i) {
      float ms = 0.f;
      HIPCHECK(hipEventElapsedTime(&ms, ev[i], ev[i + 1]));
      sum[i] += ms * 1e3;
    }
  }
  out->n = n;
  for (int i = 0; i < n; ++i) {
    out->us[i] = (float)(sum[i] / reps);
    if (std::string(st[i].name).rfind("k_pyrdown", 0) == 0) snprintf(out->name[i], sizeof(out->name[i]), "%s[%d]", st[i].name, st[i].a);
    else snprintf(out->name[i], sizeof(out->name[i]), "%s", st[i].name);
  }
  {
    std::lock_guard<std::mutex> lk(fs->edt_mu);
    fs->edt_pending = false;
    fs->ref_lists_pending = false;
    HIPCHECK(hipEventRecord(fs->ev_edt, s));
    fs->has_edt = true; fs->edt_stream = s;
    fs->has_ref = false;
  }
  HIPCHECK(hipEventRecord(fs->ev_ready, s));
  fs->has_ready = true; fs->ready_stream = s;
  for (auto& v : b->views) { v.table_built = false; v.ref_list_built = false; }
  return REVO_OK;
}

extern "C" int revo_batch_frame(revo_batch* b, int frame, revo_pyr** out) {
  if (!b || !out || frame < 0 || frame >= 2 * b->n_pairs) return fail(REVO_ERR_INVALID_ARG, "bad frame index");
  *out = &b->views[frame];
  return REVO_OK;
}

extern "C" int revo_batch_time_tracker(revo_batch* b, const float* h_init_RT, revo_pair_result* d_results, void* stream,
                                       int reps, float* ms_mean) {
  if (!b || !d_results || !ms_mean || reps <= 0) return fail(REVO_ERR_INVALID_ARG, "bad argument");
  HIPCHECK(hipSetDevice(b->ctx->device));
  hipStream_t s = stream ? (hipStream_t)stream : b->stream;
  { int rc0 = batch_wait_tracker(b, s); if (rc0) return rc0; }
  int rc = batch_upload_init(b, h_init_RT, s);
  if (rc) return rc;
  TrackParams tp = b->ctx->tp;
  tp.eval_only = 0;
  { int rc1 = batch_wait_build(b, s); if (rc1) return rc1; }
  { int rc2 = run_pending_edt(b->ctx, b->fs, s); if (rc2) return rc2; }
  float total = 0.f;
  for (int r = 0; r < reps; ++r) {
    HIPCHECK(hipEventRecord(b->ev0, s));
    rc = chained_track_launch(b->ctx->device, b->ctx->knobs.track_depth, s, [&](unsigned* d_resident) {
      return launch_track(b->d_descs, tp, d_results, nullptr, b->n_pairs, b->d_mail, &b->mail_epoch, b->cluster, d_resident, s);
    });
    if (rc) return rc;
    HIPCHECK(hipEventRecord(b->ev1, s));
    HIPCHECK(hipEventSynchronize(b->ev1));
    float ms = 0.f;
    HIPCHECK(hipEventElapsedTime(&ms, b->ev0, b->ev1));
    total += ms;
  }
  *ms_mean = total / (float)reps;
  return batch_mark_tracker(b, s);
}

struct revo_mdev {
  revo_ctx* c = nullptr;
  int S = 0, cluster = 1, hl = 0;
  TrackParams tp;
  revo_tracker_settings ts;
  FrameSet* kf = nullptr;
  std::vector<revo_pyr> kf_views;
  std::vector<FrameSet*> pool, all;
  PairDesc* h_descs = nullptr; PairDesc* d_descs = nullptr;
  revo_pair_result* d_res = nullptr; revo_pair_result* h_res = nullptr;
  unsigned long long* d_mail = nullptr;
  unsigned mail_epoch = 0;
  VoteDesc* h_vdesc = nullptr; VoteDesc* d_vdesc = nullptr;
  int* d_marks = nullptr; int* d_hist8 = nullptr; unsigned* d_done = nullptr; int* h_vout = nullptr;
  unsigned seq = 0;
  CloudCopyDesc* h_cdesc = nullptr; CloudCopyDesc* d_cdesc = nullptr;
  CopySeg* h_segs = nullptr; CopySeg* d_segs = nullptr; size_t seg_cap = 0;
  std::vector<std::deque<Past>> past;
  std::vector<Past> past_pool;
  size_t cloud_cap = 0;
  hipEvent_t ev_trk = nullptr, ev_vdesc = nullptr, ev_cdesc = nullptr, ev_segs = nullptr, ev_h2d = nullptr, ev_prod = nullptr;
};

extern "C" void revo_mdev_destroy_(revo_mdev* m) {
  if (!m) return;
  revo_ctx* c = m->c;
  hipSetDevice(c->device);
  (void)hipStreamSynchronize(c->stream);
  (void)hipStreamSynchronize(c->build_stream);
  (void)hipStreamSynchronize(c->vote_stream);
  for (FrameSet* fs : m->all) frameset_destroy(fs);
  frameset_destroy(m->kf);
  for (auto& q : m->past) for (auto& p : q) { hipFree(p.d_pts); hipFree(p.d_n); }
  for (auto& p : m->past_pool) { hipFree(p.d_pts); hipFree(p.d_n); }
  hipHostFree(m->h_descs); hipFree(m->d_descs); hipFree(m->d_res); hipHostFree(m->h_res); hipFree(m->d_mail);
  hipHostFree(m->h_vdesc); hipFree(m->d_vdesc); hipFree(m->d_marks); hipFree(m->d_hist8); hipFree(m->d_done); hipHostFree(m->h_vout);
  hipHostFree(m->h_cdesc); hipFree(m->d_cdesc); hipHostFree(m->h_segs); hipFree(m->d_segs);
  for (hipEvent_t e : {m->ev_trk, m->ev_vdesc, m->ev_cdesc, m->ev_segs, m->ev_h2d, m->ev_prod}) if (e) hipEventDestroy(e);
  (void)hipGetLastError();
  delete m;
  ctx_unref(c);
// ... 324 lines not shown
```

revo_amd/csrc/revo_pyramid.hip:

```cpp
#include "revo_dev.h"
#include <type_traits>

namespace {

#ifdef REVO_BUILD_PRIO
#define BUILD_PRIO() __builtin_amdgcn_s_setprio(REVO_BUILD_PRIO)
#else
#define BUILD_PRIO()
#endif

__device__ __forceinline__ int level_of(const PyrGeom& g, int v, int LevelGeom::*base) {
  int l = 0;
#pragma unroll
  for (int k = 1; k < REVO_L; ++k)
    if (k < g.n_levels && v >= g.lv[k].*base) l = k;
  return l;
}
__device__ __forceinline__ int clampi(int v, int lo, int hi) { return v < lo ? lo : (v > hi ? hi : v); }
__device__ __forceinline__ int reflect101(int i, int n) {
  if (i < 0) i = -i;
  if (i >= n) i = 2 * n - 2 - i;
  return i;
}

// ... 238 lines not shown
  const int x = xg * 4;
  const bool active = x < w;
  const uint8_t* gray = pl.gray[l] + (size_t)f * lv.npix;
  const bool has_prev = x > 0, has_next = x + 4 < w;
  const int xo = active ? x : 0;
  const int o_prev = (active && has_prev) ? xo - 4 : xo, o_next = (active && has_next) ? xo + 4 : xo;
  const uint32_t cm_left = (active && has_prev) ? ~0u : 0u, cm_right = (active && has_next) ? ~0u : 0u;
  struct Raw { uint32_t prev, m0, next; };
  auto load_raw = [&](int r) -> Raw {
    const int rr = clampi(r, 0, h - 1);
    const uint8_t* row = gray + (size_t)rr * w;
    Raw q;
    q.m0 = *reinterpret_cast<const uint32_t*>(row + xo);
    q.prev = *reinterpret_cast<const uint32_t*>(row + o_prev);
    q.next = *reinterpret_cast<const uint32_t*>(row + o_next);
    return q;
  };
  auto make_hrow = [&](Raw q) -> HRow4 {
    if (!has_prev) q.prev = (q.m0 & 0xffu) * 0x01010101u;
    if (!has_next) q.next = (q.m0 >> 24) * 0x01010101u;
    return hrow4(q.prev, q.m0, q.next);
  };
  HRow4 H0, H1, H2;
  MRow4 M0, M1, M2;
  DRow4 D0, D1, D2;
  {
    const Raw r0 = load_raw(y0 - 2), r1 = load_raw(y0 - 1), r2 = load_raw(y0), r3 = load_raw(y0 + 1);
    H0 = make_hrow(r0); H1 = make_hrow(r1); H2 = make_hrow(r2);
    mag_row4(H0, H1, H2, cm_left, cm_right, active && y0 - 1 >= 0, M0, D0);
    H0 = make_hrow(r3);
  }
  Raw ahead = load_raw(y0 + 2);
  mag_row4(H1, H2, H0, cm_left, cm_right, active, M1, D1);
  uint2* out = pl.cs[l] + ((size_t)f * h + y0) * lv.wpr + (xg >> 3);
  const int sh = 4 * (threadIdx.x & 7);
  auto emit = [&](int i, uint32_t cb, uint32_t sb) {
    uint32_t cw = cb << sh, sw = sb << sh;
    cw |= (uint32_t)__builtin_amdgcn_update_dpp(0, (int)cw, 0xB1, 0xf, 0xf, true);
    sw |= (uint32_t)__builtin_amdgcn_update_dpp(0, (int)sw, 0xB1, 0xf, 0xf, true);
    cw |= (uint32_t)__builtin_amdgcn_update_dpp(0, (int)cw, 0x4E, 0xf, 0xf, true);
    sw |= (uint32_t)__builtin_amdgcn_update_dpp(0, (int)sw, 0x4E, 0xf, 0xf, true);
    cw |= (uint32_t)__builtin_amdgcn_update_dpp(0, (int)cw, 0x141, 0xf, 0xf, true);
    sw |= (uint32_t)__builtin_amdgcn_update_dpp(0, (int)sw, 0x141, 0xf, 0xf, true);
    if ((threadIdx.x & 7) == 0 && y0 + i < h) out[(size_t)i * lv.wpr] = make_uint2(cw, sw);
  };
#define NMS_STEP4(i, Ha, Hb, Hc, Ma, Mb, Mc, Db, Dc)                                  \
  {                                                                                   \
    Hc = make_hrow(ahead);                                                            \
    if ((i) < NMS_R - 1) ahead = load_raw(y0 + (i) + 3);                              \
    mag_row4(Ha, Hb, Hc, cm_left, cm_right, active && y0 + (i) + 1 < h, Mc, Dc);      \
    uint32_t cb, sb;                                                                  \
    nms_row4(Ma, Mb, Mc, Db, g.canny_low, g.canny_high, &cb, &sb);                    \
    emit((i), cb, sb);                                                                \
  }
  NMS_STEP4(0, H2, H0, H1, M0, M1, M2, D1, D2)
  NMS_STEP4(1, H0, H1, H2, M1, M2, M0, D2, D0)
  NMS_STEP4(2, H1, H2, H0, M2, M0, M1, D0, D1)
  NMS_STEP4(3, H2, H0, H1, M0, M1, M2, D1, D2)
  NMS_STEP4(4, H0, H1, H2, M1, M2, M0, D2, D0)
  NMS_STEP4(5, H1, H2, H0, M2, M0, M1, D0, D1)
#undef NMS_STEP4
}

#ifndef HYST_THREADS
#define HYST_THREADS 1024
#endif
__device__ __forceinline__ uint32_t dil3(uint32_t a, uint32_t al, uint32_t ar) {
  return a | __builtin_amdgcn_alignbit(a, al, 31) | __builtin_amdgcn_alignbit(ar, a, 1);
}
__device__ __forceinline__ uint32_t run_fill(uint32_t C, uint32_t S) {
  const uint32_t up = ((C + S) ^ C) & C;
  const uint32_t rC = __builtin_bitreverse32(C), rS = __builtin_bitreverse32(S);
  const uint32_t dn = __builtin_bitreverse32(((rC + rS) ^ rC) & rC);
  return up | dn | S;
}

#ifdef REVO_HYST_PROFILE
#define HP(i) if (threadIdx.x == 0) hp[i] = clock64()
#define HA(i) if (threadIdx.x == 0) { const long long now_ = clock64(); ha[i] += now_ - hlast; hlast = now_; }
#else
#define HP(i)
#define HA(i)
#endif
template <bool C_IN_LDS, bool E_GLOBAL = false>
__device__ __forceinline__ void hyst_level(const PyrGeom& g, const FramePlanes& pl, const int l, const int f, uint32_t* s_mem) {
  static_assert(!(C_IN_LDS && E_GLOBAL), "the candidate bitmap is in LDS only when the edge bitmap is");
#ifdef REVO_HYST_PROFILE
  long long hp[12], ha[8], hlast = 0;
  for (int i = 0; i < 12; ++i) hp[i] = 0;
  for (int i = 0; i < 8; ++i) ha[i] = 0;
  int dbg_sweeps = 0, dbg_bands = 0;
#endif
  HP(0);
  const LevelGeom& lv = g.lv[l];
  const int w = lv.w, h = lv.h, wpr = lv.wpr;
  const int pitch = wpr;
  const int nwords = h * wpr;
  const int e_words = (h + 2) * pitch + 2;
  uint32_t* Cl = s_mem;
  uint32_t* Ebase = C_IN_LDS ? s_mem + (REVO_HYST_LDS_MAX / 4 - e_words)
                  : (E_GLOBAL ? reinterpret_cast<uint32_t*>(pl.scratch[l] + (size_t)f * g.lv[l].npix) : s_mem);
  uint32_t* E = Ebase + 1;
  const uint2* cs = pl.cs[l] + (size_t)f * h * wpr;
  const int tid = threadIdx.x;
  for (int i = tid; i < pitch + 1; i += HYST_THREADS) { Ebase[i] = 0u; Ebase[e_words - 1 - i] = 0u; }
  for (int i = tid; i < nwords; i += HYST_THREADS) {
    const uint2 v = cs[i];
    E[pitch + i] = v.y;
    if (C_IN_LDS) Cl[i] = v.x & ~v.y;
  }
  __syncthreads();
  HP(1);
  bool done = false;
#ifdef REVO_HYST_PROFILE
  int dbg_runs = -1, dbg_t = 0, dbg_a = 0;
#endif
  if (C_IN_LDS) {
    unsigned short* Bs = reinterpret_cast<unsigned short*>(Cl + nwords);
    uint32_t* parent = Cl + nwords + (nwords + 2) / 2;
    const int table_words = (int)(REVO_HYST_LDS_MAX / 4) - (nwords + (nwords + 2) / 2);
    const int cap = min(table_words / 2, table_words - e_words);
    const int cap_keep = (table_words - e_words) / 2;
    __shared__ int s_wsum[HYST_THREADS / 64];
    __shared__ int s_total, s_promoted;
#ifdef REVO_HYST_PROFILE
    __shared__ int s_dbg[4];
    if (tid < 4) s_dbg[tid] = 0;
#endif
    auto weak = [&](int wi) -> uint32_t { return Cl[wi]; };
    auto starts = [](uint32_t wk) -> uint32_t { return wk & ~(wk << 1); };
    const float inv_wpr = 1.0f / (float)wpr;
    const uint32_t FLAG = 0x80000000u, IDM = 0x7fffffffu;
#ifdef REVO_HYST_PROFILE
    hlast = clock64();
#endif
    for (int sweep = 0; sweep < 64 && !done; ++sweep) {
#ifdef REVO_HYST_PROFILE
      ++dbg_sweeps;
#endif
      {
        const int wpt = (nwords + HYST_THREADS - 1) / HYST_THREADS;
        const int w0 = min(nwords, tid * wpt), w1 = min(nwords, w0 + wpt);
        int mine = 0;
        for (int wi = w0; wi < w1; ++wi) mine += __popc(starts(weak(wi)));
        int incl = mine;
#pragma unroll
        for (int o = 1; o < 64; o <<= 1) {
          const int v = __shfl_up(incl, o);
          if ((tid & 63) >= o) incl += v;
        }
        __syncthreads();
        if ((tid & 63) == 63) s_wsum[tid >> 6] = incl;
        if (tid == 0) s_promoted = 0;
        __syncthreads();
        int before = incl - mine;
        for (int k = 0; k < (tid >> 6); ++k) before += s_wsum[k];
        if (tid == HYST_THREADS - 1) { s_total = before + mine; Bs[nwords] = (unsigned short)min(65535, before + mine); }
        for (int wi = w0; wi < w1; ++wi) {
          Bs[wi] = (unsigned short)before;
          before += __popc(starts(weak(wi)));
        }
        __syncthreads();
      }
      const int nruns = s_total;
      HA(0);
#ifdef REVO_HYST_PROFILE
      if (sweep == 0) dbg_runs = nruns;
// ... 144 lines not shown
    __syncthreads();
  }
  if (!done) {
    __shared__ unsigned short s_list[HYST_THREADS];
    __shared__ unsigned char s_act[2][HYST_THREADS];
    __shared__ int s_n;
  const int max_strips = HYST_THREADS / wpr;
  const int rpt = (h + max_strips - 1) / max_strips;
  const int nstrips = (h + rpt - 1) / rpt;
  const int n_items = nstrips * wpr;
  s_act[0][tid] = 0; s_act[1][tid] = 0;
  if (tid == 0) s_n = 0;
  __syncthreads();
  int n_list = n_items;
#ifndef REVO_HYST_MAXIT
#define REVO_HYST_MAXIT 8192
#endif
  for (int it = 0; it < REVO_HYST_MAXIT; ++it) {
    const int wb = it & 1;
    bool changed = false;
    if (tid < n_list) {
      const int item = it == 0 ? tid : (int)s_list[tid];
      const int strip = item / wpr, c = item - strip * wpr;
      const int r0 = strip * rpt, r1 = min(h, r0 + rpt) - 1;
      uint32_t* Ec = E + pitch + c;
      const uint32_t lm = c > 0 ? ~0u : 0u, rm = c < wpr - 1 ? ~0u : 0u;
      auto Cat = [&](int r) -> uint32_t { return C_IN_LDS ? (Cl[r * wpr + c] | Ec[r * pitch]) : cs[r * wpr + c].x; };
      uint32_t prev_d = dil3(Ec[(r0 - 1) * pitch], Ec[(r0 - 1) * pitch - 1] & lm, Ec[(r0 - 1) * pitch + 1] & rm);
      uint32_t cur = Ec[r0 * pitch], cl = Ec[r0 * pitch - 1] & lm, cr = Ec[r0 * pitch + 1] & rm;
      for (int r = r0; r <= r1; ++r) {
        const uint32_t nx = Ec[(r + 1) * pitch], nl = Ec[(r + 1) * pitch - 1] & lm, nr = Ec[(r + 1) * pitch + 1] & rm;
        const uint32_t Cw = Cat(r);
        const uint32_t hz = __builtin_amdgcn_alignbit(cur, cl, 31) | __builtin_amdgcn_alignbit(cr, cur, 1);
        const uint32_t F = run_fill(Cw, cur | (Cw & (prev_d | dil3(nx, nl, nr) | hz)));
        if (F != cur) { Ec[r * pitch] = F; changed = true; }
        prev_d = dil3(F, cl, cr);
        cur = nx; cl = nl; cr = nr;
      }
      prev_d = dil3(cur, cl, cr);
      cur = Ec[r1 * pitch]; cl = Ec[r1 * pitch - 1] & lm; cr = Ec[r1 * pitch + 1] & rm;
      for (int r = r1; r >= r0; --r) {
        const uint32_t nx = Ec[(r - 1) * pitch], nl = Ec[(r - 1) * pitch - 1] & lm, nr = Ec[(r - 1) * pitch + 1] & rm;
        const uint32_t Cw = Cat(r);
        const uint32_t hz = __builtin_amdgcn_alignbit(cur, cl, 31) | __builtin_amdgcn_alignbit(cr, cur, 1);
        const uint32_t F = run_fill(Cw, cur | (Cw & (prev_d | dil3(nx, nl, nr) | hz)));
        if (F != cur) { Ec[r * pitch] = F; changed = true; }
        prev_d = dil3(F, cl, cr);
        cur = nx; cl = nl; cr = nr;
      }
      if (changed) s_act[wb][item] = 1;
    }
    if (!__syncthreads_or(changed ? 1 : 0)) break;
    bool act = false;
    if (tid < n_items) {
      const int strip = tid / wpr, c = tid - strip * wpr;
      const unsigned char* a = s_act[wb];
#pragma unroll
      for (int ds = -1; ds <= 1; ++ds)
#pragma unroll
        for (int dc = -1; dc <= 1; ++dc) {
          const int ss = strip + ds, cc = c + dc;
          if (ss >= 0 && ss < nstrips && cc >= 0 && cc < wpr) act = act || a[ss * wpr + cc] != 0;
        }
    }
    const unsigned long long m = __ballot(act);
    int base = 0;
    if ((tid & 63) == 0 && m) base = atomicAdd(&s_n, __popcll(m));
    base = __shfl(base, 0);
    if (act) s_list[base + __popcll(m & ((1ull << (tid & 63)) - 1ull))] = (unsigned short)tid;
    s_act[wb ^ 1][tid] = 0;
    __syncthreads();
    n_list = s_n;
    __syncthreads();
    if (tid == 0) s_n = 0;
  }
  __syncthreads();
  }
  __syncthreads();
  HP(5);
  uint8_t* edges = pl.edges[l] + (size_t)f * lv.npix;
  uint8_t* orig = lv.has_orig ? pl.edges_orig[l] + (size_t)f * lv.npix : nullptr;
  const bool rows16 = (w & 15) == 0;
  const float inv_w = 1.0f / (float)w;
  for (int i = tid; i < lv.npix / 16; i += HYST_THREADS) {
    const int p = i * 16;
    int y = (int)(((float)p + 0.5f) * inv_w);
    y += (y + 1) * w <= p ? 1 : (y * w > p ? -1 : 0);
    const int x = p - y * w;
    uint32_t o[4];
    if (rows16) {
      const uint32_t bits = (E[(y + 1) * pitch + (x >> 5)] >> (x & 31)) & 0xffffu;
#pragma unroll
      for (int q = 0; q < 4; ++q) o[q] = ((((bits >> (4 * q)) & 0xfu) * 0x00204081u) & 0x01010101u) * 0xffu;
    } else {
#pragma unroll
      for (int q = 0; q < 4; ++q) {
        int xx = x + 4 * q, yy = y;
        while (xx >= w) { xx -= w; yy += 1; }
        const uint32_t bits = (E[(yy + 1) * pitch + (xx >> 5)] >> (xx & 31)) & 0xfu;
        o[q] = ((bits * 0x00204081u) & 0x01010101u) * 0xffu;
      }
    }
    const uint4 v = make_uint4(o[0], o[1], o[2], o[3]);
    *reinterpret_cast<uint4*>(edges + p) = v;
    if (orig) *reinterpret_cast<uint4*>(orig + p) = v;
  }
  {
    uint2* csw = pl.cs[l] + (size_t)f * h * wpr;
    for (int i = tid; i < nwords; i += HYST_THREADS) csw[i].y = E[pitch + i];
  }
  HP(6);
  if (lv.patch > 0) {
    const int ntiles = lv.hist_w * lv.hist_h;
    int nz = 0;
    const float inv_hw = 1.0f / (float)lv.hist_w;
    for (int t0 = 0; t0 < ntiles; t0 += HYST_THREADS) {
      const int t = t0 + tid;
      if (t < ntiles) {
        int ty = (int)(((float)t + 0.5f) * inv_hw);
        ty += (ty + 1) * lv.hist_w <= t ? 1 : (ty * lv.hist_w > t ? -1 : 0);
        const int tx = t - ty * lv.hist_w;
        const int xa = tx * lv.patch, xb = xa + lv.patch;
        const int wa = xa >> 5, wb = (xb - 1) >> 5;
        const uint32_t ma = ~0u << (xa & 31), mb = (xb & 31) ? ~0u >> (32 - (xb & 31)) : ~0u;
        const uint32_t m0 = wa == wb ? ma & mb : ma, m1 = wb > wa + 1 ? ~0u : (wb > wa ? mb : 0u), m2 = wb > wa + 1 ? mb : 0u;
        const int o1 = wb > wa ? 1 : 0, o2 = wb > wa + 1 ? 2 : 0;
        const uint32_t* row = E + (ty * lv.patch + 1) * pitch + wa;
        int cnt = 0;
        for (int y = 0; y < lv.patch; ++y, row += pitch) cnt += __popc(row[0] & m0) + __popc(row[o1] & m1) + __popc(row[o2] & m2);
        const uint8_t v = (uint8_t)(cnt & 255);
        pl.hist[l][(size_t)f * ntiles + t] = v;
        nz += v != 0;
      }
    }
    __shared__ int s_nz;
    if (tid == 0) s_nz = 0;
    __syncthreads();
    if (nz) atomicAdd(&s_nz, nz);
    __syncthreads();
    if (tid == 0) pl.hist_nz[f * REVO_L + l] = s_nz;
  }
#ifdef REVO_HYST_PROFILE
  HP(7);
  if (threadIdx.x == 0 && l == 0 && f < 64)
    printf("hyst f=%d: load %lld uf_total %lld [scan %lld record %lld link %lld compress %lld flag %lld resolve %lld] runs %d sweeps %d bands %d uf %d rebuild %lld out %lld hist %lld touched %d atomics %d\n", f,
           hp[1] - hp[0], hp[5] - hp[1], ha[0], ha[1], ha[2], ha[3], ha[4], ha[5], dbg_runs, dbg_sweeps, dbg_bands, (int)done, ha[6], hp[6] - hp[5], hp[7] - hp[6], dbg_t, dbg_a);
#endif
}
template <bool C_IN_LDS, bool E_GLOBAL = false>
__global__ void __launch_bounds__(HYST_THREADS) k_hyst(PyrGeom g, FramePlanes pl, int only_flagged, int n_frames) {
  BUILD_PRIO();
  extern __shared__ uint32_t s_mem[];
  const int n_items = g.n_levels * n_frames;
  if (only_flagged) {
    __shared__ int s_any;
    if (threadIdx.x == 0) s_any = 0;
    __syncthreads();
    for (int item = threadIdx.x; item < n_items; item += HYST_THREADS)
      if (pl.need_full[(g.frame0 + item % n_frames) * REVO_L + item / n_frames]) s_any = 1;
    __syncthreads();
    if (!s_any) return;
  }
  for (int item = blockIdx.x; item < n_items; item += gridDim.x) {
    const int l = item / n_frames;
    const int f = g.frame0 + item % n_frames;
    if (only_flagged && !pl.need_full[f * REVO_L + l]) continue;
    hyst_level<C_IN_LDS, E_GLOBAL>(g, pl, l, f, s_mem);
    __syncthreads();
  }
}

#ifndef HB_THREADS
#define HB_THREADS 1024
#endif
#ifndef HB_LDS_WORDS
#define HB_LDS_WORDS 16384
#endif
struct BandRef { int l, R0, R1; };
__device__ __forceinline__ BandRef band_ref(const PyrGeom& g, int bi) {
  int l = 0;
#pragma unroll
  for (int k = 1; k < REVO_L; ++k)
    if (k < g.n_levels && bi >= g.lv[k].band_base) l = k;
  const LevelGeom& lv = g.lv[l];
  const int b = bi - lv.band_base;
  BandRef r;
  r.l = l; r.R0 = b * lv.band_rows; r.R1 = min(lv.h, r.R0 + lv.band_rows);
  return r;
}
__device__ __forceinline__ int band_capb(const LevelGeom& lv) {
  const int hb = lv.band_rows, nwb = hb * lv.wpr;
  const int table_words = HB_LDS_WORDS - (nwb + (nwb + 2) / 2);
  const int e_words = (hb + 2) * lv.wpr + 2;
  int cap = min(table_words / 2, table_words - e_words);
  cap = min(cap, 65535);
  const int h_last = lv.h - (lv.nbands - 1) * lv.band_rows;
  cap = min(cap, ((h_last * lv.w - 4 - 2 * lv.wpr) / 8) * 5);
  return max(cap, 0) & ~31;
}
struct BandRec { int* hdr; int* bs_first; int* bs_last; uint32_t* flags; unsigned short* root; uint32_t* rec; };
__device__ __forceinline__ BandRec band_rec(const FramePlanes& pl, const LevelGeom& lv, int l, int f, int R0, int capb) {
  int* base = pl.scratch[l] + (size_t)f * lv.npix + (size_t)R0 * lv.w;
  BandRec r;
  r.hdr = base; r.bs_first = base + 4; r.bs_last = base + 4 + lv.wpr;
  r.flags = reinterpret_cast<uint32_t*>(base + 4 + 2 * lv.wpr);
  r.root = reinterpret_cast<unsigned short*>(base + 4 + 2 * lv.wpr + capb / 32);
  r.rec = reinterpret_cast<uint32_t*>(base + 4 + 2 * lv.wpr + capb / 32 + capb / 2);
  return r;
}

__device__ __forceinline__ void hyst_band(const PyrGeom& g, const FramePlanes& pl, const BandRef br, const int f, uint32_t* s_mem) {
  __shared__ int s_wsum[HB_THREADS / 64];
  __shared__ int s_total;
  const int l = br.l;
  const LevelGeom& lv = g.lv[l];
  const int h = lv.h, wpr = lv.wpr, pitch = wpr;
  const int hb = br.R1 - br.R0, nwb = hb * wpr, e_words = (hb + 2) * pitch + 2;
  const int tid = threadIdx.x;
  uint32_t* Cl = s_mem;
  uint32_t* Ebase = s_mem + (HB_LDS_WORDS - e_words);
  uint32_t* E = Ebase + 1;
  const uint2* cs = pl.cs[l] + ((size_t)f * h + br.R0) * wpr;
  const int capb = band_capb(lv);
  const BandRec rec_out = band_rec(pl, lv, l, f, br.R0, capb);
  auto load_e = [&](bool with_cl) {
    if (tid == 0) { Ebase[0] = 0u; Ebase[e_words - 1] = 0u; }
    for (int c = tid; c < wpr; c += HB_THREADS) {
      E[c] = br.R0 > 0 ? cs[c - wpr].y : 0u;
      E[(hb + 1) * pitch + c] = br.R1 < h ? cs[nwb + c].y : 0u;
    }
    for (int i0 = tid; i0 < nwb; i0 += 4 * HB_THREADS) {
      uint2 v[4];
#pragma unroll
      for (int k = 0; k < 4; ++k) v[k] = cs[min(i0 + k * HB_THREADS, nwb - 1)];
#pragma unroll
      for (int k = 0; k < 4; ++k) {
        const int i = i0 + k * HB_THREADS;
        if (i < nwb) {
          if (with_cl) { E[pitch + i] = v[k].y; Cl[i] = v[k].x & ~v[k].y; }
          else E[pitch + i] = v[k].y | (v[k].x & ~Cl[i]);
        }
      }
    }
  };
  load_e(true);
  __syncthreads();
  unsigned short* Bs = reinterpret_cast<unsigned short*>(Cl + nwb);
  uint32_t* parent = Cl + nwb + (nwb + 2) / 2;
  const int table_words = HB_LDS_WORDS - (nwb + (nwb + 2) / 2);
  const int cap_keep = (table_words - e_words) / 2;
// ... 82 lines not shown
    }
    __syncthreads();
    for (int me = tid; me < nr; me += HB_THREADS) {
      parent[me] = key_of(find(me));
      rec_out.rec[me] = rec[me];
    }
    __syncthreads();
    if (nr > cap_keep) {
      load_e(false);
      __syncthreads();
    }
    for (int wi = tid; wi < nwb; wi += HB_THREADS) {
      const uint32_t wk = Cl[wi];
      if (!wk) continue;
      int r = (int)(((float)wi + 0.5f) * inv_wpr);
      r += (r + 1) * wpr <= wi ? 1 : (r * wpr > wi ? -1 : 0);
      const int c = wi - r * wpr;
      const uint32_t lm = c > 0 ? ~0u : 0u, rm = c < wpr - 1 ? ~0u : 0u;
      const uint32_t* Xc = E + pitch + wi;
      const uint32_t sd = dil3(Xc[-pitch], Xc[-pitch - 1] & lm, Xc[-pitch + 1] & rm) | dil3(Xc[pitch], Xc[pitch - 1] & lm, Xc[pitch + 1] & rm) |
                          __builtin_amdgcn_alignbit(Xc[0], Xc[-1] & lm, 31) | __builtin_amdgcn_alignbit(Xc[1] & rm, Xc[0], 1);
      if (!(wk & sd)) continue;
      const uint32_t touched = run_fill(wk, wk & sd);
      int me = (int)Bs[wi];
      for (uint32_t m = starts(wk); m; m &= m - 1, ++me)
        if (touched & m & (0u - m)) {
          uint32_t* root = &parent[parent[me] & 0xffffu];
          if (!(*root & FLAG)) atomicOr(root, FLAG);
        }
    }
    __syncthreads();
    for (int wi = tid; wi < nwb; wi += HB_THREADS) {
      const uint32_t wk = Cl[wi];
      if (!wk) continue;
      int me = (int)Bs[wi];
      uint32_t prom = 0;
      for (uint32_t m = starts(wk); m; m &= m - 1, ++me)
        if (parent[parent[me] & 0xffffu] & FLAG) prom |= m & (0u - m);
      if (prom) E[pitch + wi] |= run_fill(wk, prom);
    }
    __syncthreads();
  }
  uint32_t* eb = pl.ebits[l] + ((size_t)f * h + br.R0) * wpr;
  for (int i = tid; i < nwb; i += HB_THREADS) eb[i] = E[pitch + i];
  if (tid == 0) { rec_out.hdr[0] = nr; rec_out.hdr[1] = 0; rec_out.hdr[2] = 1; }
  for (int c = tid; c < wpr; c += HB_THREADS) { rec_out.bs_first[c] = Bs[c]; rec_out.bs_last[c] = Bs[(hb - 1) * wpr + c]; }
  for (int i = tid; i < (nr + 31) / 32; i += HB_THREADS) {
    uint32_t bits = 0;
    for (int k = 0; k < 32; ++k) {
      const int me = 32 * i + k;
      if (me < nr && (int)(parent[me] & 0xffffu) == me && (parent[me] & FLAG)) bits |= 1u << k;
    }
    rec_out.flags[i] = bits;
  }
  for (int me = tid; me < nr; me += HB_THREADS) rec_out.root[me] = (unsigned short)(parent[me] & 0xffffu);
}
__global__ void __launch_bounds__(HB_THREADS) k_hyst_band(PyrGeom g, FramePlanes pl) {
  extern __shared__ uint32_t s_mem[];
  const int nB = gridDim.x / g.total_bands;
  hyst_band(g, pl, band_ref(g, blockIdx.x / nB), g.frame0 + blockIdx.x % nB, s_mem);
}

__device__ __forceinline__ bool hyst_frame_is_heavy(const PyrGeom& g, const FramePlanes& pl, int f) {
  __shared__ int s_cnt[HYST_THREADS / 64];
  const LevelGeom& lv = g.lv[0];
  const int nwords = lv.h * lv.wpr;
  const uint2* cs = pl.cs[0] + (size_t)f * nwords;
  int mine = 0;
  for (int i = threadIdx.x; i < nwords; i += HYST_THREADS) {
    const uint2 v = cs[i];
    const uint32_t wk = v.x & ~v.y;
    mine += __popc(wk & ~(wk << 1));
  }
#pragma unroll
  for (int o = 32; o >= 1; o >>= 1) mine += __shfl_xor(mine, o);
  __syncthreads();
  if ((threadIdx.x & 63) == 0) s_cnt[threadIdx.x >> 6] = mine;
  __syncthreads();
  int total = 0;
#pragma unroll
  for (int k = 0; k < HYST_THREADS / 64; ++k) total += s_cnt[k];
  return total >= g.hyst_heavy_runs;
}
__global__ void __launch_bounds__(HYST_THREADS) k_hyst_mixed(PyrGeom g, FramePlanes pl, int n_frames) {
  static_assert(HB_THREADS == HYST_THREADS, "one workgroup shape for both paths");
  extern __shared__ uint32_t s_mem[];
  const int nb0 = g.lv[0].nbands;
  const int n_band_wg = nb0 * n_frames;
  if ((int)blockIdx.x < n_band_wg) {
    const int f = g.frame0 + blockIdx.x % n_frames;
    if (!hyst_frame_is_heavy(g, pl, f)) return;
    hyst_band(g, pl, band_ref(g, blockIdx.x / n_frames), f, s_mem);
    return;
  }
  const int item = blockIdx.x - n_band_wg;
  const int l = item / n_frames, f = g.frame0 + item % n_frames;
  if (l == 0) {
    const bool heavy = hyst_frame_is_heavy(g, pl, f);
    if (threadIdx.x == 0) pl.hyst_heavy[f] = heavy ? 1 : 0;
    if (heavy) return;
  }
  hyst_level<true>(g, pl, l, f, s_mem);
}

#define HS_THREADS 256
#define HS_MAX_BANDS 32
#define HS_MAX_PAIRS 6144
__global__ void __launch_bounds__(HS_THREADS) k_hyst_seam(PyrGeom g, FramePlanes pl, int mixed) {
  extern __shared__ uint32_t s_fl[];
  __shared__ uint2 s_pair[HS_MAX_PAIRS];
  __shared__ int s_npairs;
  __shared__ int s_changed_band[HS_MAX_BANDS];
  const int nB = mixed ? gridDim.x : gridDim.x / g.n_levels;
  const int l = blockIdx.x / nB;
  const int f = g.frame0 + blockIdx.x % nB;
  const LevelGeom& lv = g.lv[l];
  const int nb = lv.nbands;
  if (nb <= 1 || pl.need_full[f * REVO_L + l]) return;
  if (mixed && !pl.hyst_heavy[f]) return;
  const int wpr = lv.wpr, h = lv.h;
  const int tid = threadIdx.x;
  const int capb = band_capb(lv), fw = capb / 32;
  const uint2* cs = pl.cs[l] + (size_t)f * h * wpr;
  for (int b = 0; b < nb; ++b) {
    const BandRec rb = band_rec(pl, lv, l, f, b * lv.band_rows, capb);
    const int n = (rb.hdr[0] + 31) / 32;
    for (int i = tid; i < fw; i += HS_THREADS) s_fl[b * fw + i] = i < n ? rb.flags[i] : 0u;
  }
  if (tid < HS_MAX_BANDS) s_changed_band[tid] = 0;
  if (tid == 0) s_npairs = 0;
  __syncthreads();
  auto starts = [](uint32_t wk) -> uint32_t { return wk & ~(wk << 1); };
  auto weak_at = [&](int y, int c) -> uint32_t { if (c < 0 || c >= wpr) return 0u; const uint2 v = cs[(size_t)y * wpr + c]; return v.x & ~v.y; };
  for (int item = tid; item < (nb - 1) * wpr; item += HS_THREADS) {
    const int sm = item / wpr, c = item - sm * wpr;
    const int yb = (sm + 1) * lv.band_rows, ya = yb - 1;
    const uint32_t Wa = weak_at(ya, c);
    const uint32_t Wl = weak_at(yb, c - 1), Wm = weak_at(yb, c), Wr = weak_at(yb, c + 1);
    if (!Wa || !(Wm | (Wl >> 31) | (Wr & 1u))) continue;
    const BandRec ra = band_rec(pl, lv, l, f, sm * lv.band_rows, capb);
    const BandRec rbb = band_rec(pl, lv, l, f, yb, capb);
    int ida = ra.bs_last[c];
    const int idm = rbb.bs_first[c], idl = c > 0 ? rbb.bs_first[c - 1] : 0, idr = c < wpr - 1 ? rbb.bs_first[c + 1] : 0;
    for (uint32_t m = starts(Wa); m; m &= m - 1, ++ida) {
      const int bit = __ffs(m) - 1;
      const uint32_t t2 = ~(Wa >> bit);
      const int len = t2 ? __ffs(t2) - 1 : 32 - bit;
      const uint32_t ma = (0xffffffffu >> (32 - len)) << bit;
      int roota = -1;
      for (int side = 0; side < 3; ++side) {
        int idb0; uint32_t Wb, hits;
        if (side == 0) { Wb = Wm; hits = Wm & (ma | (ma << 1) | (ma >> 1)); idb0 = idm; }
        else if (side == 1) { Wb = Wl; hits = (ma & 1u) ? (Wl & 0x80000000u) : 0u; idb0 = idl; }
        else { Wb = Wr; hits = (ma >> 31) ? (Wr & 1u) : 0u; idb0 = idr; }
        while (hits) {
          const int hb2 = __ffs(hits) - 1;
          const uint32_t upto = (2u << hb2) - 1u;
          const int k = __popc(starts(Wb) & upto) - 1;
          const uint32_t gap = ~Wb & upto;
          const int first = gap ? 32 - __clz(gap) : 0;
          const uint32_t t3 = ~(Wb >> first);
          const int lenb = t3 ? __ffs(t3) - 1 : 32 - first;
          hits &= ~((0xffffffffu >> (32 - lenb)) << first);
          if (roota < 0) roota = ra.root[ida];
          const int rootb = rbb.root[idb0 + k];
          const int slot = atomicAdd(&s_npairs, 1);
          if (slot < HS_MAX_PAIRS) s_pair[slot] = make_uint2((uint32_t)sm, (uint32_t)roota | ((uint32_t)rootb << 16));
        }
      }
    }
  }
  __syncthreads();
  const int np = s_npairs;
  if (np > HS_MAX_PAIRS) {
    if (tid == 0) pl.need_full[f * REVO_L + l] = 1;
    return;
  }
  for (int it = 0; it < 65536; ++it) {
    bool changed = false;
    for (int i = tid; i < np; i += HS_THREADS) {
      const uint2 pr = s_pair[i];
      const int sm = (int)pr.x, roota = (int)(pr.y & 0xffffu), rootb = (int)(pr.y >> 16);
      uint32_t* fa = s_fl + sm * fw;
      uint32_t* fb = s_fl + (sm + 1) * fw;
      const bool A = (fa[roota >> 5] >> (roota & 31)) & 1u, Bf = (fb[rootb >> 5] >> (rootb & 31)) & 1u;
      if (A != Bf) {
        if (!A) { atomicOr(&fa[roota >> 5], 1u << (roota & 31)); s_changed_band[sm] = 1; }
        else { atomicOr(&fb[rootb >> 5], 1u << (rootb & 31)); s_changed_band[sm + 1] = 1; }
        changed = true;
      }
    }
    if (!__syncthreads_or(changed ? 1 : 0)) break;
  }
  __syncthreads();
  for (int b = 0; b < nb; ++b) {
    if (!s_changed_band[b]) continue;
    const BandRec rb = band_rec(pl, lv, l, f, b * lv.band_rows, capb);
    const int n = (rb.hdr[0] + 31) / 32;
    for (int i = tid; i < n; i += HS_THREADS) rb.flags[i] = s_fl[b * fw + i];
    if (tid == 0) rb.hdr[1] = 1;
  }
}

#define HO_THREADS 512
__global__ void __launch_bounds__(HO_THREADS) k_hyst_out(PyrGeom g, FramePlanes pl, int mixed) {
  extern __shared__ uint32_t s_mem[];
  const int nB = gridDim.x / (mixed ? g.lv[0].nbands : g.total_bands);
  const BandRef br = band_ref(g, blockIdx.x / nB);
  const int f = g.frame0 + blockIdx.x % nB;
  const int l = br.l;
  if (pl.need_full[f * REVO_L + l]) return;
  if (mixed && !pl.hyst_heavy[f]) return;
  const LevelGeom& lv = g.lv[l];
  const int w = lv.w, h = lv.h, wpr = lv.wpr, pitch = wpr;
  const int hb = br.R1 - br.R0, nwb = hb * wpr;
  const int tid = threadIdx.x;
  uint32_t* E = s_mem;
  uint32_t* eb = pl.ebits[l] + ((size_t)f * h + br.R0) * wpr;
  for (int i = tid; i < nwb; i += HO_THREADS) E[i] = eb[i];
  const BandRec rb = band_rec(pl, lv, l, f, br.R0, band_capb(lv));
  const bool promote = rb.hdr[1] != 0;
  __syncthreads();
  if (promote) {
    const int nr = rb.hdr[0];
    for (int me = tid; me < nr; me += HO_THREADS) {
      const int root = rb.root[me];
      if ((rb.flags[root >> 5] >> (root & 31)) & 1u) {
        const uint32_t rc = rb.rec[me];
        atomicOr(&E[rc >> 10], (0xffffffffu >> (31u - (rc & 31u))) << ((rc >> 5) & 31u));
      }
    }
    __syncthreads();
  }
  uint8_t* edges = pl.edges[l] + (size_t)f * lv.npix + (size_t)br.R0 * w;
  uint8_t* orig = lv.has_orig ? pl.edges_orig[l] + (size_t)f * lv.npix + (size_t)br.R0 * w : nullptr;
  const bool rows16 = (w & 15) == 0;
  const float inv_w = 1.0f / (float)w;
  for (int i = tid; i < hb * w / 16; i += HO_THREADS) {
    const int p = i * 16;
    int y = (int)(((float)p + 0.5f) * inv_w);
    y += (y + 1) * w <= p ? 1 : (y * w > p ? -1 : 0);
    const int x = p - y * w;
    uint32_t o[4];
    if (rows16) {
      const uint32_t bits = (E[y * pitch + (x >> 5)] >> (x & 31)) & 0xffffu;
#pragma unroll
      for (int q = 0; q < 4; ++q) o[q] = ((((bits >> (4 * q)) & 0xfu) * 0x00204081u) & 0x01010101u) * 0xffu;
    } else {
#pragma unroll
      for (int q = 0; q < 4; ++q) {
        int xx = x + 4 * q, yy = y;
        while (xx >= w) { xx -= w; yy += 1; }
        const uint32_t bits = (E[yy * pitch + (xx >> 5)] >> (xx & 31)) & 0xfu;
        o[q] = ((bits * 0x00204081u) & 0x01010101u) * 0xffu;
      }
    }
    const uint4 v = make_uint4(o[0], o[1], o[2], o[3]);
    *reinterpret_cast<uint4*>(edges + p) = v;
    if (orig) *reinterpret_cast<uint4*>(orig + p) = v;
  }
  {
    uint2* csw = pl.cs[l] + ((size_t)f * h + br.R0) * wpr;
    for (int i = tid; i < nwb; i += HO_THREADS) csw[i].y = E[i];
  }
  if (lv.patch > 0) {
    const int ty0 = br.R0 / lv.patch, ty1 = min(lv.hist_h, br.R1 / lv.patch);
    const int ntiles = max(0, ty1 - ty0) * lv.hist_w;
    int nz = 0;
    for (int t = tid; t < ntiles; t += HO_THREADS) {
      const int ty = ty0 + t / lv.hist_w, tx = t % lv.hist_w;
      const int xa = tx * lv.patch, xb = xa + lv.patch;
      const int wa = xa >> 5, wb = (xb - 1) >> 5;
      const uint32_t ma = ~0u << (xa & 31), mb = (xb & 31) ? ~0u >> (32 - (xb & 31)) : ~0u;
      const uint32_t m0 = wa == wb ? ma & mb : ma, m1 = wb > wa + 1 ? ~0u : (wb > wa ? mb : 0u), m2 = wb > wa + 1 ? mb : 0u;
      const int o1 = wb > wa ? 1 : 0, o2 = wb > wa + 1 ? 2 : 0;
      const uint32_t* row = E + (ty * lv.patch - br.R0) * pitch + wa;
      int cnt = 0;
      for (int y = 0; y < lv.patch; ++y, row += pitch) cnt += __popc(row[0] & m0) + __popc(row[o1] & m1) + __popc(row[o2] & m2);
      const uint8_t v = (uint8_t)(cnt & 255);
      pl.hist[l][(size_t)f * lv.hist_w * lv.hist_h + (size_t)ty * lv.hist_w + tx] = v;
      nz += v != 0;
    }
#pragma unroll
    for (int o = 32; o > 0; o >>= 1) nz += __shfl_xor(nz, o);
    if ((tid & 63) == 0 && nz) atomicAdd(&pl.hist_nz[f * REVO_L + l], nz);
  }
}

__global__ void __launch_bounds__(1024) k_fill(PyrGeom g, FramePlanes pl, int only_level) {
  BUILD_PRIO();
  const int f = g.frame0 + blockIdx.z;
  const int la = only_level ? only_level : 1, lb = only_level ? only_level + 1 : g.n_levels;
  for (int l = la; l < lb; ++l) {
    const LevelGeom lv = g.lv[l], lf = g.lv[l - 1];
    if (!(g.use_edge_hist && lv.patch > 0 && lf.patch > 0)) continue;
    const float frac = (float)pl.hist_nz[f * REVO_L + l] / (float)(lv.hist_w * lv.hist_h);
    if (frac < g.n_percentage) {
      const uint8_t* top = pl.edges[l - 1] + (size_t)f * lf.npix;
      uint8_t* mod = pl.edges[l] + (size_t)f * lv.npix;
      const uint8_t* hist = pl.hist[l] + (size_t)f * lv.hist_w * lv.hist_h;
      const double thr = g.fill_thr[l];
      const int cw = lf.w / 2, ch = lf.h / 2;
      for (int i = blockIdx.x * 1024 + threadIdx.x; i < cw * ch; i += gridDim.x * 1024) {
        const int y = i / cw, x = i % cw;
        const int yy = 2 * y + 1, xx = 2 * x + 1;
        const int ty = yy / lf.patch, tx = xx / lf.patch;
        if (ty >= lv.hist_h || tx >= lv.hist_w) continue;
        if ((double)hist[(size_t)ty * lv.hist_w + tx] < thr && top[(size_t)yy * lf.w + xx] > 0) {
          mod[(size_t)y * lv.w + x] = 255;
          atomicOr(&(pl.cs[l] + (size_t)f * lv.h * lv.wpr)[(size_t)y * lv.wpr + (x >> 5)].y, 1u << (x & 31));
        }
      }
    }
    __syncthreads();
  }
}

__device__ __forceinline__ uint32_t tile_transpose32(uint32_t v, int r) {
#pragma unroll
  for (int k = 16; k >= 1; k >>= 1) {
    const uint32_t mk = k == 16 ? 0x0000ffffu : k == 8 ? 0x00ff00ffu : k == 4 ? 0x0f0f0f0fu : k == 2 ? 0x33333333u : 0x55555555u;
    const uint32_t t = (uint32_t)__shfl_xor((int)v, k);
    v = (r & k) ? ((v & ~mk) | ((t >> k) & mk)) : ((v & mk) | ((t & mk) << k));
  }
  return v;
}

__device__ __forceinline__ bool depth_ok(float Z, float dmin, float dmax) {
  return isfinite(Z) && Z > dmin && Z < dmax;
}

#define CW_COLS 64
#define CW_LANES 16
#ifndef CW_LANES_COUNT
#define CW_LANES_COUNT 8
#endif
#define CW_MAXCHUNK 64
#define CW_STAGE 4096
template <bool WRITE>
__global__ void __launch_bounds__(CW_COLS * (WRITE ? CW_LANES : CW_LANES_COUNT)) k_compact_walk(PyrGeom g, FramePlanes pl) {
  constexpr int LANES = WRITE ? CW_LANES : CW_LANES_COUNT;
  __shared__ int s_cnt[CW_COLS * CW_MAXCHUNK];
  __shared__ unsigned s_mask[CW_COLS * CW_MAXCHUNK];
  __shared__ float4 s_pts[WRITE ? CW_STAGE : 1];
  const int nB = gridDim.x / g.total_strips;
  const int sx = blockIdx.x / nB;
  const int f = g.frame0 + blockIdx.x % nB;
  const int l = level_of(g, sx, &LevelGeom::strip_base);
  const LevelGeom& lv = g.lv[l];
  const int strip = sx - lv.strip_base;
  const int tid = threadIdx.x, xl = tid & (CW_COLS - 1), cl = tid / CW_COLS;
  const int x = strip * CW_COLS + xl;
  const int ncols = min(CW_COLS, lv.w - strip * CW_COLS);
  const int nslots = ncols * lv.nchunk;
  const size_t slot0 = (size_t)f * lv.w * lv.nchunk + (size_t)strip * CW_COLS * lv.nchunk;
  const float* depth = pl.depth[l] + (size_t)f * lv.npix;
  if (!WRITE) {
    const uint8_t* edges = pl.edges[l] + (size_t)f * lv.npix;
    const bool bit_tiles = l < g.n_levels - 1 && (lv.w & 31) == 0 && lv.chunk_rows == 32;
    if (bit_tiles) {
      const uint2* csw = pl.cs[l] + (size_t)f * lv.h * lv.wpr;
      const uint32_t* vw = reinterpret_cast<const uint32_t*>(pl.vb[l] + (size_t)f * (lv.npix >> 3));
      const int lane = tid & 63, r = lane & 31;
      const int wc = strip * (CW_COLS / 32) + (lane >> 5);
      for (int c = cl; c < lv.nchunk; c += LANES) {
        const int y = c * 32 + r;
        uint32_t v = 0;
        if (y < lv.h && wc < lv.wpr) v = csw[(size_t)y * lv.wpr + wc].y & vw[(size_t)y * lv.wpr + wc];
        v = tile_transpose32(v, r);
        if (x < lv.w) {
          s_mask[xl * lv.nchunk + c] = v;
          s_cnt[xl * lv.nchunk + c] = __popc(v);
        }
      }
    } else
    if (x < lv.w) {
      for (int c = cl; c < lv.nchunk; c += LANES) {
        const int yb = c * lv.chunk_rows, ye = min(lv.h, yb + lv.chunk_rows);
        unsigned em = 0;
#pragma unroll 8
        for (int y = yb; y < ye; ++y) em |= (edges[(size_t)y * lv.w + x] ? 1u : 0u) << (y - yb);
        unsigned vm = 0;
        if (l < g.n_levels - 1) {
          const uint8_t* vb = pl.vb[l] + (size_t)f * (lv.npix >> 3);
          const int vpitch = lv.w >> 3;
          if (em) {
#pragma unroll 8
            for (int y = yb; y < ye; ++y) vm |= ((unsigned)(vb[(size_t)y * vpitch + (x >> 3)] >> (x & 7)) & 1u) << (y - yb);
            vm &= em;
          }
        } else
        for (unsigned m = em; m;) {
          int b[4];
          float Z[4];
#pragma unroll
          for (int j = 0; j < 4; ++j) {
            b[j] = m ? __ffs(m) - 1 : -1;
            m &= m - 1;
// ... 348 lines not shown
  const int i = blockIdx.x * 256 + threadIdx.x;
  if (i >= dw * dh) return;
  const int x = i % dw, y = i / dw;
  const int kk[5] = {1, 4, 6, 4, 1};
  int acc[3] = {0, 0, 0};
#pragma unroll
  for (int j = 0; j < 5; ++j) {
    const uint8_t* row = src + (size_t)reflect101(2 * y + j - 2, h) * w * 3;
    int rs[3] = {0, 0, 0};
#pragma unroll
    for (int t = 0; t < 5; ++t) {
      const uint8_t* px = row + (size_t)reflect101(2 * x + t - 2, w) * 3;
      rs[0] += kk[t] * px[0]; rs[1] += kk[t] * px[1]; rs[2] += kk[t] * px[2];
    }
    acc[0] += kk[j] * rs[0]; acc[1] += kk[j] * rs[1]; acc[2] += kk[j] * rs[2];
  }
  uint8_t* o = dst + (size_t)i * 3;
  o[0] = (uint8_t)((acc[0] + 128) >> 8); o[1] = (uint8_t)((acc[1] + 128) >> 8); o[2] = (uint8_t)((acc[2] + 128) >> 8);
}

template <bool WRITE>
__global__ void __launch_bounds__(256) k_pcl_walk(LevelGeom lv, float dmin, float dmax, const float* __restrict__ depth,
                                                  const uint8_t* __restrict__ edges, const uint8_t* __restrict__ bgr,
                                                  int dense, int* __restrict__ chunk, unsigned* __restrict__ cmask,
                                                  const int* __restrict__ total, int cap, float4* __restrict__ out) {
  const int i = blockIdx.x * 256 + threadIdx.x;
  if (i >= lv.w * lv.nchunk) return;
  const int x = i % lv.w, c = i / lv.w;
  const int yb = c * lv.chunk_rows, ye = min(lv.h, yb + lv.chunk_rows);
  const size_t slot = (size_t)x * lv.nchunk + c;
  if (!WRITE) {
    unsigned vm = 0;
    for (int y = yb; y < ye; ++y) {
      const size_t p = (size_t)y * lv.w + x;
      if ((dense || edges[p]) && depth_ok(depth[p], dmin, dmax)) vm |= 1u << (y - yb);
    }
    cmask[slot] = vm;
    chunk[slot] = __popc(vm);
  } else {
    if (*total > cap) return;
    int o = chunk[slot];
    for (unsigned m = cmask[slot]; m; m &= m - 1) {
      const int y = yb + __ffs(m) - 1;
      const size_t p = (size_t)y * lv.w + x;
      const float Z = depth[p];
      const float X = __fdiv_rn(Z * ((float)x - lv.cx), lv.fx);
      const float Y = __fdiv_rn(Z * ((float)y - lv.cy), lv.fy);
      const uint8_t* px = bgr + p * 3;
      out[2 * o] = make_float4(X, Y, Z, 1.0f);
      out[2 * o + 1] = make_float4(__fdiv_rn((float)px[2], 255.0f), __fdiv_rn((float)px[1], 255.0f),
                                   __fdiv_rn((float)px[0], 255.0f), 1.0f);
      ++o;
    }
  }
}

__global__ void __launch_bounds__(1024) k_pcl_scan(int* chunk, int n, int* total) {
  __shared__ int s_part[1024];
  const int t = block_exclusive_scan(chunk, n, s_part);
  if (threadIdx.x == 0) *total = t;
}

#define EDT_INF (1 << 29)
#define EDT_THREADS 1024
#define EDT_COL_GROUPS(h) ((h) > 1024 ? 64 : ((h) > 512 ? 32 : 16))
__global__ void __launch_bounds__(EDT_THREADS) k_edt_cols(PyrGeom g, FramePlanes pl, int f0, int fstride, int nframes) {
  __shared__ int s_first[EDT_THREADS];
  __shared__ int s_last[EDT_THREADS];
  const int f = f0 + (blockIdx.x % nframes) * fstride;
  int l = 0, sidx = blockIdx.x / nframes, ngroups = 16, ncols = 64;
  for (int k = 0; k < g.n_levels; ++k) {
    ngroups = EDT_COL_GROUPS(g.lv[k].h);
    ncols = EDT_THREADS / ngroups;
    const int ns = (g.lv[k].w + ncols - 1) / ncols;
    if (sidx < ns) { l = k; break; }
    sidx -= ns;
  }
  const LevelGeom& lv = g.lv[l];
  const int col = threadIdx.x % ncols, grp = threadIdx.x / ncols;
  const int x = sidx * ncols + col;
  const int rpg = (lv.h + ngroups - 1) / ngroups;
  const int yb = min(lv.h, grp * rpg), ye = min(lv.h, yb + rpg);
  const bool in = x < lv.w;
  const uint8_t* edges = pl.edges[l] + (size_t)f * lv.npix;
  unsigned em = 0;
  if ((lv.w & 31) == 0 && (ncols & 31) == 0) {
    const uint2* csw = pl.cs[l] + (size_t)f * lv.h * lv.wpr;
    const int r = threadIdx.x & 31;
    const int wc = (sidx * ncols + (col & ~31)) >> 5;
    uint32_t v = 0;
    if (yb + r < ye && wc < lv.wpr) v = csw[(size_t)(yb + r) * lv.wpr + wc].y;
    em = tile_transpose32(v, r);
    if (!in) em = 0;
  } else if (in) {
#pragma unroll 8
    for (int y = yb; y < ye; ++y) em |= (edges[(size_t)y * lv.w + x] ? 1u : 0u) << (y - yb);
  }
  s_first[grp * ncols + col] = em ? yb + __ffs(em) - 1 : EDT_INF;
  s_last[grp * ncols + col] = em ? yb + 31 - __clz(em) : -EDT_INF;
  __syncthreads();
  if (!in) return;
  int above = -EDT_INF, below = EDT_INF;
  for (int k = 0; k < grp; ++k) above = max(above, s_last[k * ncols + col]);
  for (int k = ngroups - 1; k > grp; --k) below = min(below, s_first[k * ncols + col]);
  uint16_t* gd = reinterpret_cast<uint16_t*>(pl.scratch[l]) + (size_t)f * lv.npix;
  const int FAR = 1 << 20;
  int du = (above <= -EDT_INF) ? FAR : (yb - above);
  const int dbelow = (below >= EDT_INF) ? FAR : (below - yb);
  for (int y = yb; y < ye; ++y) {
    const int k = y - yb;
    const unsigned hi = em >> k;
    du = (hi & 1u) ? 0 : du;
    const int dn = hi ? __ffs(hi) - 1 : dbelow - k;
    const int m = min(du, dn);
    gd[(size_t)y * lv.w + x] = (uint16_t)(m >= 0xffff ? 0xffff : m);
    du += 1;
  }
}

__device__ __forceinline__ float sqrt_rn_int(float x) {
  const float s = __builtin_amdgcn_sqrtf(x);
  const unsigned si = __float_as_uint(s);
  const float sd = __uint_as_float(si - 1u), su = __uint_as_float(si + 1u);
  const float rd = __builtin_fmaf(-sd, s, x), ru = __builtin_fmaf(-su, s, x);
  float r = (rd <= 0.0f) ? sd : s;
  r = (ru > 0.0f) ? su : r;
  return r;
}
__global__ void __launch_bounds__(256) k_edt_rows(PyrGeom g, FramePlanes pl, int f0, int fstride) {
  extern __shared__ int s_g2[];
  const int f = f0 + blockIdx.z * fstride;
  const int l = level_of(g, blockIdx.x, &LevelGeom::edt_block_base);
  const LevelGeom lv = g.lv[l];
  const int w = lv.w;
  const int y0 = (blockIdx.x - lv.edt_block_base) * lv.edt_rows;
  const int nr = min(lv.edt_rows, lv.h - y0);
  const int pad = w + 4, pitch = w + 2 * pad;
  const uint16_t* gd = reinterpret_cast<const uint16_t*>(pl.scratch[l]) + (size_t)f * lv.npix + (size_t)y0 * w;
  const int4 inf4 = make_int4(EDT_INF, EDT_INF, EDT_INF, EDT_INF);
  const int padq = pad >> 2, wq = w >> 2;
  for (int r = 0; r < nr; ++r) {
    int4* row4 = reinterpret_cast<int4*>(s_g2 + r * pitch);
    for (int i = threadIdx.x; i < padq; i += 256) { row4[i] = inf4; row4[padq + wq + i] = inf4; }
    const uint2* src = reinterpret_cast<const uint2*>(gd + r * w);
    for (int i = threadIdx.x; i < wq; i += 256) {
      const uint2 q = src[i];
      const int d0 = (int)(q.x & 0xffffu), d1 = (int)(q.x >> 16), d2 = (int)(q.y & 0xffffu), d3 = (int)(q.y >> 16);
      row4[padq + i] = make_int4(d0 == 0xffff ? EDT_INF : __mul24(d0, d0), d1 == 0xffff ? EDT_INF : __mul24(d1, d1),
                                 d2 == 0xffff ? EDT_INF : __mul24(d2, d2), d3 == 0xffff ? EDT_INF : __mul24(d3, d3));
    }
  }
  __syncthreads();
  float* dt = pl.dt[l] + (size_t)f * lv.npix + (size_t)y0 * w;
  const int dq = 256 / w, dr = 256 - dq * w;
  int r = threadIdx.x / w, x = threadIdx.x - r * w;
  for (int p = threadIdx.x; p < nr * w; p += 256) {
    const int* c = s_g2 + r * pitch + pad + x;
    int best = c[0];
    for (int d = 1; d < w && d * d < best; d += 4) {
      int m = best;
#pragma unroll
      for (int j = 0; j < 4; ++j) {
        const int dj = d + j;
        m = min(m, dj * dj + min(c[-dj], c[dj]));
      }
      best = m;
    }
    dt[p] = best >= EDT_INF ? sqrtf(1e15f) : sqrt_rn_int((float)best);
    x += dr; r += dq;
    if (x >= w) { x -= w; ++r; }
  }
}

__global__ void __launch_bounds__(256) k_grad_table(PyrGeom g, FramePlanes pl, int f0, int fstride) {
  const int f = f0 + blockIdx.z * fstride;
  const int l = blockIdx.y;
  const LevelGeom& lv = g.lv[l];
  const int i = blockIdx.x * 256 + threadIdx.x;
  if (i >= lv.npix) return;
// ... 100 lines not shown
    if (m) marks[i] = 0;
    const float Z = d.depth[i];
    if (depth_ok(Z, dmin, dmax)) {
      const int val = __popc(m);
      atomicAdd(&s_h[val], 1);
      if (d.edges[i] > 0) atomicAdd(&s_h[4 + val], 1);
    }
  }
  __syncthreads();
  if (threadIdx.x < 8 && s_h[threadIdx.x]) atomicAdd(&d.hist8[threadIdx.x], s_h[threadIdx.x]);
  __threadfence();
  __syncthreads();
  if (threadIdx.x == 0) s_last = (atomicAdd(d.done, 1u) == gridDim.x - 1);
  __syncthreads();
  if (s_last) {
    if (threadIdx.x < 8) d.host_out[threadIdx.x] = atomicExch(&d.hist8[threadIdx.x], 0);
    if (threadIdx.x == 0) *d.done = 0u;
    __threadfence_system();
    __syncthreads();
    if (threadIdx.x == 0) *(volatile int*)&d.host_out[8] = (int)seq_val;
  }
}

__global__ void __launch_bounds__(256) k_copy_cloud_multi(const CloudCopyDesc* __restrict__ descs) {
  const CloudCopyDesc& d = descs[blockIdx.y];
  const int n = *d.src_n;
  for (int i = blockIdx.x * 256 + threadIdx.x; i < n; i += gridDim.x * 256) d.dst[i] = d.src[i];
  if (blockIdx.x == 0 && threadIdx.x == 0) *d.dst_n = n;
}

__global__ void __launch_bounds__(256) k_copy_segments(const CopySeg* __restrict__ segs) {
  const CopySeg& sg = segs[blockIdx.y];
  const char* src = (const char*)sg.src;
  char* dst = (char*)sg.dst;
  const size_t bytes = sg.bytes;
  const size_t step = (size_t)gridDim.x * 256;
  if ((((uintptr_t)src | (uintptr_t)dst | bytes) & 15) == 0) {
    const uint4* s4 = (const uint4*)src;
    uint4* d4 = (uint4*)dst;
    for (size_t i = blockIdx.x * 256 + threadIdx.x; i < bytes / 16; i += step) d4[i] = s4[i];
  } else {
    for (size_t i = blockIdx.x * 256 + threadIdx.x; i < bytes; i += step) dst[i] = src[i];
  }
}

}

void launch_gray_depth(const PyrGeom& g, const FramePlanes& p, const uint8_t* d_bgr, const float* d_depth_f32,
                       const uint16_t* d_depth_u16, float u16_alpha, int B, hipStream_t s) {
  const int npix = g.lv[0].npix;
  dim3 grid((npix / 16 + 255) / 256, 1, B);
  hipLaunchKernelGGL(k_gray_depth, grid, dim3(256), 0, s, d_bgr, d_depth_f32, d_depth_u16, u16_alpha, p.gray[0],
                     p.depth[0], npix, g.frame0);
}

void launch_pyrdown(const PyrGeom& g, const FramePlanes& p, int lvl, int B, hipStream_t s, int parts, bool stage_edges) {
  const LevelGeom& d = g.lv[lvl];
  const LevelGeom& sl = g.lv[lvl - 1];
  dim3 grid(((d.w / 4) * ((d.h + 1) / 2) + 255) / 256, 1, B);
  EdgeStage es{};
  if (stage_edges) {
    int tb = 0;
    for (int k = 0; k < lvl - 1; ++k) tb += g.lv[k].wpr * g.lv[k].nchunk;
    es.cs = p.cs[lvl - 1]; es.epre = p.epre[lvl - 1]; es.base = p.stage_base + tb; es.out = p.stage[lvl - 1];
    es.wpr = sl.wpr; es.tiles_total = g.total_tiles;
  }
#define PYRDOWN_ARGS p.gray[lvl - 1], sl.w, sl.h, p.gray[lvl], d.w, d.h, p.depth[lvl - 1], p.depth[lvl], g.frame0, g.fstride, p.vb[lvl - 1], g.depth_min, g.depth_max, es
  if (parts == 1) hipLaunchKernelGGL((k_pyrdown<true, false>), grid, dim3(256), 0, s, PYRDOWN_ARGS);
  else if (parts == 2 && stage_edges) hipLaunchKernelGGL((k_pyrdown<false, true, true>), grid, dim3(256), 0, s, PYRDOWN_ARGS);
  else if (parts == 2) hipLaunchKernelGGL((k_pyrdown<false, true>), grid, dim3(256), 0, s, PYRDOWN_ARGS);
  else hipLaunchKernelGGL((k_pyrdown<true, true>), grid, dim3(256), 0, s, PYRDOWN_ARGS);
#undef PYRDOWN_ARGS
}

void launch_edge_prefix(const PyrGeom& g, const FramePlanes& p, int B, hipStream_t s) {
  if (g.n_levels < 2) return;
  hipLaunchKernelGGL(k_edge_prefix, dim3((g.n_levels - 1) * B), dim3(1024), 0, s, g, p);
}

void launch_canny_nms(const PyrGeom& g, const FramePlanes& p, int B, hipStream_t s) {
  hipLaunchKernelGGL(k_canny_nms4, dim3(g.total_nms_blocks, 1, B), dim3(256), 0, s, g, p);
}

void launch_hyst(const PyrGeom& g, const FramePlanes& p, int B, hipStream_t s) {
  size_t e_bytes = 0, ec_bytes = 0;
  for (int l = 0; l < g.n_levels; ++l) {
    const size_t nw = (size_t)g.lv[l].h * g.lv[l].wpr;
    const size_t e = ((size_t)(g.lv[l].h + 2) * g.lv[l].wpr + 2) * 4, c = (nw + (nw + 2) / 2) * 4;
    e_bytes = e > e_bytes ? e : e_bytes;
    ec_bytes = e + c > ec_bytes ? e + c : ec_bytes;
  }
  static bool attr_set = false;
  if (!attr_set) {
    (void)hipFuncSetAttribute(reinterpret_cast<const void*>(k_hyst<true>), hipFuncAttributeMaxDynamicSharedMemorySize, REVO_HYST_LDS_MAX);
    (void)hipFuncSetAttribute(reinterpret_cast<const void*>(k_hyst<false>), hipFuncAttributeMaxDynamicSharedMemorySize, REVO_HYST_LDS_MAX);
    attr_set = true;
  }
  const int force = g.hyst_force;
  const bool fits_single = ec_bytes + 4096 <= REVO_HYST_LDS_MAX;
  const bool banded = force >= 0 ? force == 1 : !fits_single;
  const int only_flagged = banded && g.total_bands > 0 ? 1 : 0;
  if (only_flagged) {
    static bool attr2 = false;
    if (!attr2) {
      (void)hipFuncSetAttribute(reinterpret_cast<const void*>(k_hyst_band), hipFuncAttributeMaxDynamicSharedMemorySize, HB_LDS_WORDS * 4);
      (void)hipFuncSetAttribute(reinterpret_cast<const void*>(k_hyst_out), hipFuncAttributeMaxDynamicSharedMemorySize, HB_LDS_WORDS * 4);
      (void)hipFuncSetAttribute(reinterpret_cast<const void*>(k_hyst_seam), hipFuncAttributeMaxDynamicSharedMemorySize, 64 * 1024);
      (void)hipGetLastError();
      attr2 = true;
    }
    size_t seam_lds = 4, out_lds = 4;
    for (int l = 0; l < g.n_levels; ++l) {
      const LevelGeom& lv = g.lv[l];
      const size_t nwb = (size_t)lv.band_rows * lv.wpr;
      out_lds = std::max(out_lds, nwb * 4);
      if (lv.nbands > 1) seam_lds = std::max(seam_lds, (size_t)lv.nbands * (size_t)(HB_LDS_WORDS / 2 / 32 + 64) * 4);
    }
    hipLaunchKernelGGL(k_hyst_band, dim3(g.total_bands * B), dim3(HB_THREADS), HB_LDS_WORDS * 4, s, g, p);
    if (g.any_banded) hipLaunchKernelGGL(k_hyst_seam, dim3(g.n_levels * B), dim3(HS_THREADS), seam_lds, s, g, p, 0);
    hipLaunchKernelGGL(k_hyst_out, dim3(g.total_bands * B), dim3(HO_THREADS), out_lds, s, g, p, 0);
  }
  const bool mixed = !banded && fits_single && g.hyst_heavy_runs > 0 && g.total_bands > 0 && g.lv[0].nbands > 1;
  if (mixed) {
    static bool attr3 = false;
    if (!attr3) {
      (void)hipFuncSetAttribute(reinterpret_cast<const void*>(k_hyst_mixed), hipFuncAttributeMaxDynamicSharedMemorySize, REVO_HYST_LDS_MAX);
      (void)hipFuncSetAttribute(reinterpret_cast<const void*>(k_hyst_out), hipFuncAttributeMaxDynamicSharedMemorySize, HB_LDS_WORDS * 4);
      (void)hipFuncSetAttribute(reinterpret_cast<const void*>(k_hyst_seam), hipFuncAttributeMaxDynamicSharedMemorySize, 64 * 1024);
      (void)hipGetLastError();
      attr3 = true;
    }
    const LevelGeom& l0 = g.lv[0];
    const size_t seam_lds = std::max<size_t>(4, (size_t)l0.nbands * (size_t)(HB_LDS_WORDS / 2 / 32 + 64) * 4);
    const size_t out_lds = std::max<size_t>(4, (size_t)l0.band_rows * l0.wpr * 4);
    hipLaunchKernelGGL(k_hyst_mixed, dim3((l0.nbands + g.n_levels) * B), dim3(HYST_THREADS), REVO_HYST_LDS_MAX, s, g, p, B);
    hipLaunchKernelGGL(k_hyst_seam, dim3(B), dim3(HS_THREADS), seam_lds, s, g, p, 1);
    hipLaunchKernelGGL(k_hyst_out, dim3(l0.nbands * B), dim3(HO_THREADS), out_lds, s, g, p, 1);
    hipLaunchKernelGGL(k_hyst<true>, dim3(std::min(32, g.n_levels * B)), dim3(HYST_THREADS), REVO_HYST_LDS_MAX, s, g, p, 1, B);
    return;
  }
  const int n_wg = only_flagged ? std::min(32, g.n_levels * B) : g.n_levels * B;
  if (ec_bytes + 4096 <= REVO_HYST_LDS_MAX)
    hipLaunchKernelGGL(k_hyst<true>, dim3(n_wg), dim3(HYST_THREADS), REVO_HYST_LDS_MAX, s, g, p, only_flagged, B);
  else if (e_bytes <= REVO_HYST_LDS_MAX)
    hipLaunchKernelGGL(k_hyst<false>, dim3(n_wg), dim3(HYST_THREADS), e_bytes, s, g, p, only_flagged, B);
  else
    hipLaunchKernelGGL((k_hyst<false, true>), dim3(n_wg), dim3(HYST_THREADS), 16, s, g, p, only_flagged, B);
}

void launch_fill(const PyrGeom& g, const FramePlanes& p, int B, hipStream_t s) {
  bool any = false;
  for (int l = 1; l < g.n_levels; ++l) any = any || g.lv[l].has_orig;
  if (!any) return;
  if (g.lv[0].npix <= 640 * 480) {
    hipLaunchKernelGGL(k_fill, dim3(1, 1, B), dim3(1024), 0, s, g, p, 0);
    return;
  }
  for (int l = 1; l < g.n_levels; ++l) {
    if (!g.lv[l].has_orig) continue;
    const int n = (g.lv[l - 1].w / 2) * (g.lv[l - 1].h / 2);
    hipLaunchKernelGGL(k_fill, dim3(std::min(64, (n + 1023) / 1024), 1, B), dim3(1024), 0, s, g, p, l);
  }
}

void launch_tile_points(const PyrGeom& g, const FramePlanes& p, int B, hipStream_t s, int which) {
  if (which & 1) hipLaunchKernelGGL(k_tile_count, dim3(g.n_levels * B), dim3(1024), 0, s, g, p);
  const int groups = (g.total_tiles + PT_TILES - 1) / PT_TILES;
  if ((which & 2) && g.pts_staged) hipLaunchKernelGGL(k_pts_tiles<true>, dim3(groups * B), dim3(32 * PT_TILES), 0, s, g, p);
  else if (which & 2) hipLaunchKernelGGL(k_pts_tiles<false>, dim3(groups * B), dim3(32 * PT_TILES), 0, s, g, p);
}

void launch_compact(const PyrGeom& g, const FramePlanes& p, int B, hipStream_t s) {
  dim3 grid(g.total_strips * B);
  hipLaunchKernelGGL(k_compact_walk<false>, grid, dim3(CW_COLS * CW_LANES_COUNT), 0, s, g, p);
  hipLaunchKernelGGL(k_compact_walk<true>, grid, dim3(CW_COLS * CW_LANES), 0, s, g, p);
}

void launch_pyrdown_bgr(const uint8_t* src, int w, int h, uint8_t* dst, hipStream_t s) {
  hipLaunchKernelGGL(k_pyrdown_bgr, dim3(((w / 2) * (h / 2) + 255) / 256), dim3(256), 0, s, src, w, h, dst);
}

void launch_colored_pcl(const PyrGeom& g, const FramePlanes& p, int frame, int lvl, int dense, const uint8_t* bgr_lvl,
                        int* chunk, unsigned* cmask, int* total, int cap, float* out8, hipStream_t s) {
  const LevelGeom& lv = g.lv[lvl];
  const float* depth = p.depth[lvl] + (size_t)frame * lv.npix;
  const uint8_t* edges = p.edges[lvl] + (size_t)frame * lv.npix;
  const int n = lv.w * lv.nchunk;
  dim3 grid((n + 255) / 256);
  hipLaunchKernelGGL(k_pcl_walk<false>, grid, dim3(256), 0, s, lv, g.depth_min, g.depth_max, depth, edges, bgr_lvl, dense,
                     chunk, cmask, total, cap, (float4*)out8);
  hipLaunchKernelGGL(k_pcl_scan, dim3(1), dim3(1024), 0, s, chunk, n, total);
  hipLaunchKernelGGL(k_pcl_walk<true>, grid, dim3(256), 0, s, lv, g.depth_min, g.depth_max, depth, edges, bgr_lvl, dense,
                     chunk, cmask, total, cap, (float4*)out8);
}

void launch_keyframe(const PyrGeom& g, const FramePlanes& p, int f0, int fstride, int count, hipStream_t s, int which) {
  int strips = 0;
  for (int l = 0; l < g.n_levels; ++l) {
    const int ncols = EDT_THREADS / EDT_COL_GROUPS(g.lv[l].h);
    strips += (g.lv[l].w + ncols - 1) / ncols;
  }
  if (which & 1) hipLaunchKernelGGL(k_edt_cols, dim3(strips * count), dim3(EDT_THREADS), 0, s, g, p, f0, fstride, count);
  size_t rows_lds = 0;
  for (int l = 0; l < g.n_levels; ++l) rows_lds = std::max(rows_lds, (size_t)g.lv[l].edt_rows * (3 * g.lv[l].w + 8) * sizeof(int));
  if (which & 2) hipLaunchKernelGGL(k_edt_rows, dim3(g.total_edt_blocks, 1, count), dim3(256), rows_lds, s, g, p, f0, fstride);
}

void launch_grad_table(const PyrGeom& g, const FramePlanes& p, int f0, int fstride, int count, hipStream_t s) {
  hipLaunchKernelGGL(k_grad_table, dim3((g.lv[0].npix + 255) / 256, g.n_levels, count), dim3(256), 0, s, g, p, f0, fstride);
}

void launch_vote(const PyrGeom& g, const FramePlanes& curr, int curr_frame, int lvl, int n_clouds, const VoteArgs& va,
                 int* d_marks, int* d_hist8, unsigned* d_done, int* h_out8, unsigned seq_val, int use_orig_edges, hipStream_t s) {
  const LevelGeom& lv = g.lv[lvl];
  if (n_clouds > 0)
    hipLaunchKernelGGL(k_vote_mark, dim3(32, n_clouds), dim3(256), 0, s, va, lv.fx, lv.fy, lv.cx, lv.cy, lv.w, lv.h, d_marks);
  const uint8_t* edges = (use_orig_edges ? curr.edges_orig[lvl] : curr.edges[lvl]) + (size_t)curr_frame * lv.npix;
  hipLaunchKernelGGL(k_vote_hist, dim3(16), dim3(256), 0, s, d_marks, edges,
                     curr.depth[lvl] + (size_t)curr_frame * lv.npix, lv.npix, g.depth_min, g.depth_max, d_hist8, d_done, h_out8,
                     seq_val);
}

void launch_copy_cloud(float4* dst, const float4* src, int* dst_n, const int* src_n, hipStream_t s) {
  hipLaunchKernelGGL(k_copy_cloud, dim3(16), dim3(256), 0, s, dst, src, dst_n, src_n);
}

void launch_vote_multi(const PyrGeom& g, int lvl, int n, const VoteDesc* d_descs, unsigned seq_val, hipStream_t s) {
  const LevelGeom& lv = g.lv[lvl];
  hipLaunchKernelGGL(k_vote_mark_multi, dim3(32, 3, n), dim3(256), 0, s, d_descs, lv.fx, lv.fy, lv.cx, lv.cy, lv.w, lv.h);
  hipLaunchKernelGGL(k_vote_hist_multi, dim3(16, n), dim3(256), 0, s, d_descs, lv.npix, g.depth_min, g.depth_max, seq_val);
}

void launch_copy_cloud_multi(int n, const CloudCopyDesc* d_descs, hipStream_t s) {
  hipLaunchKernelGGL(k_copy_cloud_multi, dim3(16, n), dim3(256), 0, s, d_descs);
}

void launch_copy_segments(int n, const CopySeg* d_segs, hipStream_t s) {
  hipLaunchKernelGGL(k_copy_segments, dim3(64, n), dim3(256), 0, s, d_segs);
}
```

Measured before the change: 114,400.

## Defer byte edge-plane expansion until a consumer needs it

```diff
diff --git a/include/revo_hip.h b/include/revo_hip.h
--- a/include/revo_hip.h
+++ b/include/revo_hip.h
@@ -347,6 +347,7 @@
 int revo_debug_gate_timeouts_(int device);
 void revo_debug_section_max_(unsigned long long out[12], int reset);
 void revo_debug_wait_stats_(unsigned long long out[3]);
+unsigned long long revo_debug_plane_expansions_(void);
 int revo_debug_track_profile_(revo_ctx* ctx, float out13[13]);
 int revo_debug_batch_profile_(float* out, int n_pairs);
 
diff --git a/revo_amd/csrc/revo_dev.h b/revo_amd/csrc/revo_dev.h
--- a/revo_amd/csrc/revo_dev.h
+++ b/revo_amd/csrc/revo_dev.h
@@ -125,8 +125,9 @@
 void launch_pyrdown(const PyrGeom& g, const FramePlanes& p, int lvl, int B, hipStream_t s, int parts = 3, bool stage_edges = false);
 void launch_edge_prefix(const PyrGeom& g, const FramePlanes& p, int B, hipStream_t s);
 void launch_canny_nms(const PyrGeom& g, const FramePlanes& p, int B, hipStream_t s);
-void launch_hyst(const PyrGeom& g, const FramePlanes& p, int B, hipStream_t s);
-void launch_fill(const PyrGeom& g, const FramePlanes& p, int B, hipStream_t s);
+void launch_hyst(const PyrGeom& g, const FramePlanes& p, int B, hipStream_t s, bool bytes = true);
+void launch_fill(const PyrGeom& g, const FramePlanes& p, int B, hipStream_t s, bool bytes = true);
+void launch_expand_edges(const PyrGeom& g, const FramePlanes& p, int B, hipStream_t s);
 void launch_compact(const PyrGeom& g, const FramePlanes& p, int B, hipStream_t s);
 void launch_tile_points(const PyrGeom& g, const FramePlanes& p, int B, hipStream_t s, int which = 3);
 void launch_pyrdown_bgr(const uint8_t* src, int w, int h, uint8_t* dst, hipStream_t s);
diff --git a/revo_amd/csrc/revo_host.hip b/revo_amd/csrc/revo_host.hip
--- a/revo_amd/csrc/revo_host.hip
+++ b/revo_amd/csrc/revo_host.hip
@@ -69,6 +69,10 @@
   hipEvent_t ev_ref = nullptr;
   hipStream_t ref_stream = nullptr;
   bool has_ref = false;
+  std::atomic<bool> planes_pending{false};
+  hipEvent_t ev_planes = nullptr;
+  hipStream_t planes_stream = nullptr;
+  bool has_planes = false;
   hipEvent_t ev_free = nullptr;
   hipEvent_t ev_free2 = nullptr;
   hipEvent_t ev_h2d = nullptr;
@@ -405,6 +409,7 @@
   HIPCHECK(hipEventCreateWithFlags(&fs->ev_free2, hipEventDisableTiming));
   HIPCHECK(hipEventCreateWithFlags(&fs->ev_edt, hipEventDisableTiming));
   HIPCHECK(hipEventCreateWithFlags(&fs->ev_ref, hipEventDisableTiming));
+  HIPCHECK(hipEventCreateWithFlags(&fs->ev_planes, hipEventDisableTiming));
   hipMemsetAsync(fs->p.npts, 0, sizeof(int) * REVO_L * B, c->stream);
   HIPCHECK(hipStreamSynchronize(c->stream));
   *out = fs;
@@ -420,6 +425,7 @@
   if (fs->ev_free2) hipEventDestroy(fs->ev_free2);
   if (fs->ev_edt) hipEventDestroy(fs->ev_edt);
   if (fs->ev_ref) hipEventDestroy(fs->ev_ref);
+  if (fs->ev_planes) hipEventDestroy(fs->ev_planes);
   if (fs->ev_h2d) hipEventDestroy(fs->ev_h2d);
   delete fs;
 }
@@ -434,8 +440,8 @@
   launch_gray_depth(g, fs->p, d_bgr, d_depth_f32, d_depth_u16, alpha, B, s);
   for (int l = 1; l < g.n_levels; ++l) launch_pyrdown(g, fs->p, l, B, s, gray_only ? 1 : 3);
   launch_canny_nms(g, fs->p, B, s);
-  launch_hyst(g, fs->p, B, s);
-  launch_fill(g, fs->p, B, s);
+  launch_hyst(g, fs->p, B, s, !gray_only);
+  launch_fill(g, fs->p, B, s, !gray_only);
   if (with_points) launch_tile_points(g, fs->p, B, s);
 }
 
@@ -628,10 +634,29 @@
   fs->ref_lists_pending = false;
   return REVO_OK;
 }
+static std::atomic<unsigned long long> g_plane_expansions{0};
+extern "C" unsigned long long revo_debug_plane_expansions_() { return g_plane_expansions.load(); }
+static int materialize_planes(revo_ctx* c, FrameSet* fs, hipStream_t s) {
+  std::lock_guard<std::mutex> lk(fs->edt_mu);
+  if (!fs->planes_pending) {
+    if (fs->has_planes && fs->planes_stream != s) HIPCHECK(hipStreamWaitEvent(s, fs->ev_planes, 0));
+    return REVO_OK;
+  }
+  if (fs->has_ready) HIPCHECK(hipStreamWaitEvent(s, fs->ev_ready, 0));
+  launch_expand_edges(c->geom, fs->p, fs->B, s);
+  HIPCHECK(hipGetLastError());
+  g_plane_expansions.fetch_add(1, std::memory_order_relaxed);
+  HIPCHECK(hipEventRecord(fs->ev_planes, s));
+  fs->has_planes = true;
+  fs->planes_stream = s;
+  fs->planes_pending = false;
+  return REVO_OK;
+}
 static int wait_edt_before_rebuild(FrameSet* fs, hipStream_t s) {
   std::lock_guard<std::mutex> lk(fs->edt_mu);
   if (fs->has_edt && fs->edt_stream != s) HIPCHECK(hipStreamWaitEvent(s, fs->ev_edt, 0));
   if (fs->has_ref && fs->ref_stream != s) HIPCHECK(hipStreamWaitEvent(s, fs->ev_ref, 0));
+  if (fs->has_planes && fs->planes_stream != s) HIPCHECK(hipStreamWaitEvent(s, fs->ev_planes, 0));
   return REVO_OK;
 }
 typedef unsigned v4u __attribute__((ext_vector_type(4)));
@@ -694,11 +719,12 @@
   HIPCHECK(hipEventSynchronize(ev));
   return REVO_OK;
 }
-static int wait_ready_on(revo_ctx* c, const revo_pyr* p, hipStream_t s) {
+static int wait_ready_on(revo_ctx* c, const revo_pyr* p, hipStream_t s, bool need_planes = false) {
   if (p->fs->has_ready) HIPCHECK(hipStreamWaitEvent(s, p->fs->ev_ready, 0));
-  return run_pending_edt(c, p->fs, s, (p->frame & 1) == 0);
-}
-static int wait_ready(revo_ctx* c, const revo_pyr* p) { return wait_ready_on(c, p, c->stream); }
+  { int rc = run_pending_edt(c, p->fs, s, (p->frame & 1) == 0); if (rc) return rc; }
+  return need_planes ? materialize_planes(c, p->fs, s) : REVO_OK;
+}
+static int wait_ready(revo_ctx* c, const revo_pyr* p, bool need_planes = false) { return wait_ready_on(c, p, c->stream, need_planes); }
 static int vote_enqueued(revo_ctx* c, const revo_pyr* p) {
   if (p->owns_fs) return REVO_OK;
   HIPCHECK(hipEventRecord(c->ev_vote, c->vote_stream));
@@ -842,7 +868,8 @@
   const LevelGeom& v = c->geom.lv[lvl];
   const FramePlanes& P = p->fs->p;
   const size_t f = (size_t)p->frame;
-  { int rc = wait_ready(c, p); if (rc) return rc; }
+  const bool planes = what == REVO_PLANE_EDGES || what == REVO_PLANE_EDGES_ORIG || what == REVO_PLANE_EDGES3D;
+  { int rc = wait_ready(c, p, planes); if (rc) return rc; }
   HIPCHECK(hipStreamSynchronize(c->stream));
   const void* src = nullptr;
   size_t n = v.npix, esz = 1;
@@ -903,7 +930,7 @@
   if (lvl < 0 || lvl >= c->geom.n_levels) return fail(REVO_ERR_LEVEL, "level out of range");
   if (!(p->owns_fs || p->has_colour) || !p->fs->d_bgr)
     return fail(REVO_ERR_INVALID_ARG, "batch views keep no colour image (rgbFullSize): use revo_pyramid_create");
-  { int rc = wait_ready(c, p); if (rc) return rc; }
+  { int rc = wait_ready(c, p, true); if (rc) return rc; }
   std::lock_guard<std::mutex> lk(c->mu);
   const PyrGeom& g = c->geom;
   const size_t n0 = g.lv[0].npix, slots = (size_t)g.lv[0].w * g.lv[0].nchunk;
@@ -945,7 +972,7 @@
   HIPCHECK(hipSetDevice(c->device));
   if (!(p->owns_fs || p->has_colour) || !p->fs->d_bgr)
     return fail(REVO_ERR_INVALID_ARG, "batch views keep no colour image (rgbFullSize): use revo_pyramid_create");
-  { int rc = wait_ready(c, p); if (rc) return rc; }
+  { int rc = wait_ready(c, p, true); if (rc) return rc; }
   const size_t n0 = c->geom.lv[0].npix, f = (size_t)p->frame;
   out->ctx = c;
   out->depth = p->fs->p.depth[0] + f * n0;
@@ -1143,7 +1170,7 @@
   const int hl = c->ts.histogram_level;
   if (hl < 0 || hl >= c->geom.n_levels) return fail(REVO_ERR_LEVEL, "histogram_level outside the pyramid");
   hipStream_t vs = c->vote_stream;
-  { int rc = wait_ready_on(c, curr, vs); if (rc) return rc; }
+  { int rc = wait_ready_on(c, curr, vs, true); if (rc) return rc; }
   float inv[16];
   mat4_inverse(T_w_curr, inv);
   int nframes = 0;
@@ -1361,6 +1388,7 @@
     std::lock_guard<std::mutex> lk(b->fs->edt_mu);
     b->fs->edt_pending = true; b->fs->edt_count = b->n_pairs;
     b->fs->ref_lists_pending = true;
+    b->fs->planes_pending = true;
   } else {
     launch_tile_points(g, b->fs->p, b->fs->B, s);
     launch_keyframe(g, b->fs->p, 0, 2, b->n_pairs, s);
@@ -1739,6 +1767,7 @@
     HIPCHECK(hipEventRecord(fs->ev_edt, s));
     fs->has_edt = true; fs->edt_stream = s;
     fs->has_ref = false;
+    fs->planes_pending = false;
   }
   HIPCHECK(hipEventRecord(fs->ev_ready, s));
   fs->has_ready = true; fs->ready_stream = s;
diff --git a/revo_amd/csrc/revo_pyramid.hip b/revo_amd/csrc/revo_pyramid.hip
--- a/revo_amd/csrc/revo_pyramid.hip
+++ b/revo_amd/csrc/revo_pyramid.hip
@@ -344,7 +344,7 @@
 #define HP(i)
 #define HA(i)
 #endif
-template <bool C_IN_LDS, bool E_GLOBAL = false>
+template <bool C_IN_LDS, bool E_GLOBAL = false, bool BYTES = true>
 __device__ __forceinline__ void hyst_level(const PyrGeom& g, const FramePlanes& pl, const int l, const int f, uint32_t* s_mem) {
   static_assert(!(C_IN_LDS && E_GLOBAL), "the candidate bitmap is in LDS only when the edge bitmap is");
 #ifdef REVO_HYST_PROFILE
@@ -655,6 +655,7 @@
   uint8_t* orig = lv.has_orig ? pl.edges_orig[l] + (size_t)f * lv.npix : nullptr;
   const bool rows16 = (w & 15) == 0;
   const float inv_w = 1.0f / (float)w;
+  if (BYTES)
   for (int i = tid; i < lv.npix / 16; i += HYST_THREADS) {
     const int p = i * 16;
     int y = (int)(((float)p + 0.5f) * inv_w);
@@ -681,6 +682,10 @@
   {
     uint2* csw = pl.cs[l] + (size_t)f * h * wpr;
     for (int i = tid; i < nwords; i += HYST_THREADS) csw[i].y = E[pitch + i];
+    if (!BYTES && lv.has_orig) {
+      uint32_t* eb = pl.ebits[l] + (size_t)f * h * wpr;
+      for (int i = tid; i < nwords; i += HYST_THREADS) eb[i] = E[pitch + i];
+    }
   }
   HP(6);
   if (lv.patch > 0) {
@@ -720,7 +725,7 @@
            hp[1] - hp[0], hp[5] - hp[1], ha[0], ha[1], ha[2], ha[3], ha[4], ha[5], dbg_runs, dbg_sweeps, dbg_bands, (int)done, ha[6], hp[6] - hp[5], hp[7] - hp[6], dbg_t, dbg_a);
 #endif
 }
-template <bool C_IN_LDS, bool E_GLOBAL = false>
+template <bool C_IN_LDS, bool E_GLOBAL = false, bool BYTES = true>
 __global__ void __launch_bounds__(HYST_THREADS) k_hyst(PyrGeom g, FramePlanes pl, int only_flagged, int n_frames) {
   BUILD_PRIO();
   extern __shared__ uint32_t s_mem[];
@@ -738,7 +743,7 @@
     const int l = item / n_frames;
     const int f = g.frame0 + item % n_frames;
     if (only_flagged && !pl.need_full[f * REVO_L + l]) continue;
-    hyst_level<C_IN_LDS, E_GLOBAL>(g, pl, l, f, s_mem);
+    hyst_level<C_IN_LDS, E_GLOBAL, BYTES>(g, pl, l, f, s_mem);
     __syncthreads();
   }
 }
@@ -987,6 +992,7 @@
   for (int k = 0; k < HYST_THREADS / 64; ++k) total += s_cnt[k];
   return total >= g.hyst_heavy_runs;
 }
+template <bool BYTES>
 __global__ void __launch_bounds__(HYST_THREADS) k_hyst_mixed(PyrGeom g, FramePlanes pl, int n_frames) {
   static_assert(HB_THREADS == HYST_THREADS, "one workgroup shape for both paths");
   extern __shared__ uint32_t s_mem[];
@@ -1005,7 +1011,7 @@
     if (threadIdx.x == 0) pl.hyst_heavy[f] = heavy ? 1 : 0;
     if (heavy) return;
   }
-  hyst_level<true>(g, pl, l, f, s_mem);
+  hyst_level<true, false, BYTES>(g, pl, l, f, s_mem);
 }
 
 #define HS_THREADS 256
@@ -1108,6 +1114,7 @@
 }
 
 #define HO_THREADS 512
+template <bool BYTES>
 __global__ void __launch_bounds__(HO_THREADS) k_hyst_out(PyrGeom g, FramePlanes pl, int mixed) {
   extern __shared__ uint32_t s_mem[];
   const int nB = gridDim.x / (mixed ? g.lv[0].nbands : g.total_bands);
@@ -1141,6 +1148,7 @@
   uint8_t* orig = lv.has_orig ? pl.edges_orig[l] + (size_t)f * lv.npix + (size_t)br.R0 * w : nullptr;
   const bool rows16 = (w & 15) == 0;
   const float inv_w = 1.0f / (float)w;
+  if (BYTES)
   for (int i = tid; i < hb * w / 16; i += HO_THREADS) {
     const int p = i * 16;
     int y = (int)(((float)p + 0.5f) * inv_w);
@@ -1167,6 +1175,8 @@
   {
     uint2* csw = pl.cs[l] + ((size_t)f * h + br.R0) * wpr;
     for (int i = tid; i < nwb; i += HO_THREADS) csw[i].y = E[i];
+    if (!BYTES && lv.has_orig)
+      for (int i = tid; i < nwb; i += HO_THREADS) eb[i] = E[i];
   }
   if (lv.patch > 0) {
     const int ty0 = br.R0 / lv.patch, ty1 = min(lv.hist_h, br.R1 / lv.patch);
@@ -1192,6 +1202,7 @@
   }
 }
 
+template <bool BYTES>
 __global__ void __launch_bounds__(1024) k_fill(PyrGeom g, FramePlanes pl, int only_level) {
   BUILD_PRIO();
   const int f = g.frame0 + blockIdx.z;
@@ -1204,6 +1215,10 @@
       const uint8_t* top = pl.edges[l - 1] + (size_t)f * lf.npix;
       uint8_t* mod = pl.edges[l] + (size_t)f * lv.npix;
       const uint8_t* hist = pl.hist[l] + (size_t)f * lv.hist_w * lv.hist_h;
+      uint2* topw = pl.cs[l - 1] + (size_t)f * lf.h * lf.wpr;
+      auto top_bit = [&](int yy, int xx) -> bool {
+        return (__hip_atomic_load(&topw[(size_t)yy * lf.wpr + (xx >> 5)].y, __ATOMIC_RELAXED, __HIP_MEMORY_SCOPE_AGENT) >> (xx & 31)) & 1u;
+      };
       const double thr = g.fill_thr[l];
       const int cw = lf.w / 2, ch = lf.h / 2;
       for (int i = blockIdx.x * 1024 + threadIdx.x; i < cw * ch; i += gridDim.x * 1024) {
@@ -1211,14 +1226,31 @@
         const int yy = 2 * y + 1, xx = 2 * x + 1;
         const int ty = yy / lf.patch, tx = xx / lf.patch;
         if (ty >= lv.hist_h || tx >= lv.hist_w) continue;
-        if ((double)hist[(size_t)ty * lv.hist_w + tx] < thr && top[(size_t)yy * lf.w + xx] > 0) {
-          mod[(size_t)y * lv.w + x] = 255;
+        if ((double)hist[(size_t)ty * lv.hist_w + tx] < thr && (BYTES ? top[(size_t)yy * lf.w + xx] > 0 : top_bit(yy, xx))) {
+          if (BYTES) mod[(size_t)y * lv.w + x] = 255;
           atomicOr(&(pl.cs[l] + (size_t)f * lv.h * lv.wpr)[(size_t)y * lv.wpr + (x >> 5)].y, 1u << (x & 31));
         }
       }
     }
     __syncthreads();
   }
+}
+
+__global__ void __launch_bounds__(256) k_expand_edges(PyrGeom g, FramePlanes pl) {
+  const int q = blockIdx.x * 256 + threadIdx.x;
+  if (q >= g.total_pix / 4) return;
+  const int f = g.frame0 + blockIdx.y;
+  int l = 0;
+#pragma unroll
+  for (int k = 1; k < REVO_L; ++k)
+    if (k < g.n_levels && 4 * q >= g.lv[k].pix_base) l = k;
+  const LevelGeom& lv = g.lv[l];
+  const int p = 4 * q - lv.pix_base;
+  const int y = p / lv.w, x = p - y * lv.w;
+  const size_t wi = ((size_t)f * lv.h + y) * lv.wpr + (x >> 5);
+  auto bytes4 = [&](uint32_t word) -> uint32_t { return ((((word >> (x & 31)) & 0xfu) * 0x00204081u) & 0x01010101u) * 0xffu; };
+  *reinterpret_cast<uint32_t*>(pl.edges[l] + (size_t)f * lv.npix + p) = bytes4(pl.cs[l][wi].y);
+  if (lv.has_orig) *reinterpret_cast<uint32_t*>(pl.edges_orig[l] + (size_t)f * lv.npix + p) = bytes4(pl.ebits[l][wi]);
 }
 
 __device__ __forceinline__ uint32_t tile_transpose32(uint32_t v, int r) {
@@ -1733,10 +1765,9 @@
   const int rpg = (lv.h + ngroups - 1) / ngroups;
   const int yb = min(lv.h, grp * rpg), ye = min(lv.h, yb + rpg);
   const bool in = x < lv.w;
-  const uint8_t* edges = pl.edges[l] + (size_t)f * lv.npix;
+  const uint2* csw = pl.cs[l] + (size_t)f * lv.h * lv.wpr;
   unsigned em = 0;
-  if ((lv.w & 31) == 0 && (ncols & 31) == 0) {
-    const uint2* csw = pl.cs[l] + (size_t)f * lv.h * lv.wpr;
+  if ((ncols & 31) == 0) {
     const int r = threadIdx.x & 31;
     const int wc = (sidx * ncols + (col & ~31)) >> 5;
     uint32_t v = 0;
@@ -1745,7 +1776,7 @@
     if (!in) em = 0;
   } else if (in) {
 #pragma unroll 8
-    for (int y = yb; y < ye; ++y) em |= (edges[(size_t)y * lv.w + x] ? 1u : 0u) << (y - yb);
+    for (int y = yb; y < ye; ++y) em |= ((csw[(size_t)y * lv.wpr + (x >> 5)].y >> (x & 31)) & 1u) << (y - yb);
   }
   s_first[grp * ncols + col] = em ? yb + __ffs(em) - 1 : EDT_INF;
   s_last[grp * ncols + col] = em ? yb + 31 - __clz(em) : -EDT_INF;
@@ -2012,7 +2043,7 @@
   hipLaunchKernelGGL(k_canny_nms4, dim3(g.total_nms_blocks, 1, B), dim3(256), 0, s, g, p);
 }
 
-void launch_hyst(const PyrGeom& g, const FramePlanes& p, int B, hipStream_t s) {
+void launch_hyst(const PyrGeom& g, const FramePlanes& p, int B, hipStream_t s, bool bytes) {
   size_t e_bytes = 0, ec_bytes = 0;
   for (int l = 0; l < g.n_levels; ++l) {
     const size_t nw = (size_t)g.lv[l].h * g.lv[l].wpr;
@@ -2024,6 +2055,8 @@
   if (!attr_set) {
     (void)hipFuncSetAttribute(reinterpret_cast<const void*>(k_hyst<true>), hipFuncAttributeMaxDynamicSharedMemorySize, REVO_HYST_LDS_MAX);
     (void)hipFuncSetAttribute(reinterpret_cast<const void*>(k_hyst<false>), hipFuncAttributeMaxDynamicSharedMemorySize, REVO_HYST_LDS_MAX);
+    (void)hipFuncSetAttribute(reinterpret_cast<const void*>((k_hyst<true, false, false>)), hipFuncAttributeMaxDynamicSharedMemorySize, REVO_HYST_LDS_MAX);
+    (void)hipFuncSetAttribute(reinterpret_cast<const void*>((k_hyst<false, false, false>)), hipFuncAttributeMaxDynamicSharedMemorySize, REVO_HYST_LDS_MAX);
     attr_set = true;
   }
   const int force = g.hyst_force;
@@ -2034,7 +2067,8 @@
     static bool attr2 = false;
     if (!attr2) {
       (void)hipFuncSetAttribute(reinterpret_cast<const void*>(k_hyst_band), hipFuncAttributeMaxDynamicSharedMemorySize, HB_LDS_WORDS * 4);
-      (void)hipFuncSetAttribute(reinterpret_cast<const void*>(k_hyst_out), hipFuncAttributeMaxDynamicSharedMemorySize, HB_LDS_WORDS * 4);
+      (void)hipFuncSetAttribute(reinterpret_cast<const void*>(k_hyst_out<true>), hipFuncAttributeMaxDynamicSharedMemorySize, HB_LDS_WORDS * 4);
+      (void)hipFuncSetAttribute(reinterpret_cast<const void*>(k_hyst_out<false>), hipFuncAttributeMaxDynamicSharedMemorySize, HB_LDS_WORDS * 4);
       (void)hipFuncSetAttribute(reinterpret_cast<const void*>(k_hyst_seam), hipFuncAttributeMaxDynamicSharedMemorySize, 64 * 1024);
       (void)hipGetLastError();
       attr2 = true;
@@ -2048,14 +2082,17 @@
     }
     hipLaunchKernelGGL(k_hyst_band, dim3(g.total_bands * B), dim3(HB_THREADS), HB_LDS_WORDS * 4, s, g, p);
     if (g.any_banded) hipLaunchKernelGGL(k_hyst_seam, dim3(g.n_levels * B), dim3(HS_THREADS), seam_lds, s, g, p, 0);
-    hipLaunchKernelGGL(k_hyst_out, dim3(g.total_bands * B), dim3(HO_THREADS), out_lds, s, g, p, 0);
+    if (bytes) hipLaunchKernelGGL(k_hyst_out<true>, dim3(g.total_bands * B), dim3(HO_THREADS), out_lds, s, g, p, 0);
+    else hipLaunchKernelGGL(k_hyst_out<false>, dim3(g.total_bands * B), dim3(HO_THREADS), out_lds, s, g, p, 0);
   }
   const bool mixed = !banded && fits_single && g.hyst_heavy_runs > 0 && g.total_bands > 0 && g.lv[0].nbands > 1;
   if (mixed) {
     static bool attr3 = false;
     if (!attr3) {
-      (void)hipFuncSetAttribute(reinterpret_cast<const void*>(k_hyst_mixed), hipFuncAttributeMaxDynamicSharedMemorySize, REVO_HYST_LDS_MAX);
-      (void)hipFuncSetAttribute(reinterpret_cast<const void*>(k_hyst_out), hipFuncAttributeMaxDynamicSharedMemorySize, HB_LDS_WORDS * 4);
+      (void)hipFuncSetAttribute(reinterpret_cast<const void*>(k_hyst_mixed<true>), hipFuncAttributeMaxDynamicSharedMemorySize, REVO_HYST_LDS_MAX);
+      (void)hipFuncSetAttribute(reinterpret_cast<const void*>(k_hyst_mixed<false>), hipFuncAttributeMaxDynamicSharedMemorySize, REVO_HYST_LDS_MAX);
+      (void)hipFuncSetAttribute(reinterpret_cast<const void*>(k_hyst_out<true>), hipFuncAttributeMaxDynamicSharedMemorySize, HB_LDS_WORDS * 4);
+      (void)hipFuncSetAttribute(reinterpret_cast<const void*>(k_hyst_out<false>), hipFuncAttributeMaxDynamicSharedMemorySize, HB_LDS_WORDS * 4);
       (void)hipFuncSetAttribute(reinterpret_cast<const void*>(k_hyst_seam), hipFuncAttributeMaxDynamicSharedMemorySize, 64 * 1024);
       (void)hipGetLastError();
       attr3 = true;
@@ -2063,34 +2100,48 @@
     const LevelGeom& l0 = g.lv[0];
     const size_t seam_lds = std::max<size_t>(4, (size_t)l0.nbands * (size_t)(HB_LDS_WORDS / 2 / 32 + 64) * 4);
     const size_t out_lds = std::max<size_t>(4, (size_t)l0.band_rows * l0.wpr * 4);
-    hipLaunchKernelGGL(k_hyst_mixed, dim3((l0.nbands + g.n_levels) * B), dim3(HYST_THREADS), REVO_HYST_LDS_MAX, s, g, p, B);
+    const dim3 gm((l0.nbands + g.n_levels) * B), go(l0.nbands * B), gd(std::min(32, g.n_levels * B));
+    if (bytes) hipLaunchKernelGGL(k_hyst_mixed<true>, gm, dim3(HYST_THREADS), REVO_HYST_LDS_MAX, s, g, p, B);
+    else hipLaunchKernelGGL(k_hyst_mixed<false>, gm, dim3(HYST_THREADS), REVO_HYST_LDS_MAX, s, g, p, B);
     hipLaunchKernelGGL(k_hyst_seam, dim3(B), dim3(HS_THREADS), seam_lds, s, g, p, 1);
-    hipLaunchKernelGGL(k_hyst_out, dim3(l0.nbands * B), dim3(HO_THREADS), out_lds, s, g, p, 1);
-    hipLaunchKernelGGL(k_hyst<true>, dim3(std::min(32, g.n_levels * B)), dim3(HYST_THREADS), REVO_HYST_LDS_MAX, s, g, p, 1, B);
+    if (bytes) hipLaunchKernelGGL(k_hyst_out<true>, go, dim3(HO_THREADS), out_lds, s, g, p, 1);
+    else hipLaunchKernelGGL(k_hyst_out<false>, go, dim3(HO_THREADS), out_lds, s, g, p, 1);
+    if (bytes) hipLaunchKernelGGL(k_hyst<true>, gd, dim3(HYST_THREADS), REVO_HYST_LDS_MAX, s, g, p, 1, B);
+    else hipLaunchKernelGGL((k_hyst<true, false, false>), gd, dim3(HYST_THREADS), REVO_HYST_LDS_MAX, s, g, p, 1, B);
     return;
   }
   const int n_wg = only_flagged ? std::min(32, g.n_levels * B) : g.n_levels * B;
-  if (ec_bytes + 4096 <= REVO_HYST_LDS_MAX)
-    hipLaunchKernelGGL(k_hyst<true>, dim3(n_wg), dim3(HYST_THREADS), REVO_HYST_LDS_MAX, s, g, p, only_flagged, B);
-  else if (e_bytes <= REVO_HYST_LDS_MAX)
-    hipLaunchKernelGGL(k_hyst<false>, dim3(n_wg), dim3(HYST_THREADS), e_bytes, s, g, p, only_flagged, B);
-  else
-    hipLaunchKernelGGL((k_hyst<false, true>), dim3(n_wg), dim3(HYST_THREADS), 16, s, g, p, only_flagged, B);
-}
-
-void launch_fill(const PyrGeom& g, const FramePlanes& p, int B, hipStream_t s) {
+#define HYST_LAUNCH(KERNEL, lds) hipLaunchKernelGGL(KERNEL, dim3(n_wg), dim3(HYST_THREADS), lds, s, g, p, only_flagged, B)
+  if (ec_bytes + 4096 <= REVO_HYST_LDS_MAX) {
+    if (bytes) HYST_LAUNCH(k_hyst<true>, REVO_HYST_LDS_MAX); else HYST_LAUNCH((k_hyst<true, false, false>), REVO_HYST_LDS_MAX);
+  } else if (e_bytes <= REVO_HYST_LDS_MAX) {
+    if (bytes) HYST_LAUNCH(k_hyst<false>, e_bytes); else HYST_LAUNCH((k_hyst<false, false, false>), e_bytes);
+  } else {
+    if (bytes) HYST_LAUNCH((k_hyst<false, true>), 16); else HYST_LAUNCH((k_hyst<false, true, false>), 16);
+  }
+#undef HYST_LAUNCH
+}
+
+void launch_fill(const PyrGeom& g, const FramePlanes& p, int B, hipStream_t s, bool bytes) {
   bool any = false;
   for (int l = 1; l < g.n_levels; ++l) any = any || g.lv[l].has_orig;
   if (!any) return;
   if (g.lv[0].npix <= 640 * 480) {
-    hipLaunchKernelGGL(k_fill, dim3(1, 1, B), dim3(1024), 0, s, g, p, 0);
+    if (bytes) hipLaunchKernelGGL(k_fill<true>, dim3(1, 1, B), dim3(1024), 0, s, g, p, 0);
+    else hipLaunchKernelGGL(k_fill<false>, dim3(1, 1, B), dim3(1024), 0, s, g, p, 0);
     return;
   }
   for (int l = 1; l < g.n_levels; ++l) {
     if (!g.lv[l].has_orig) continue;
     const int n = (g.lv[l - 1].w / 2) * (g.lv[l - 1].h / 2);
-    hipLaunchKernelGGL(k_fill, dim3(std::min(64, (n + 1023) / 1024), 1, B), dim3(1024), 0, s, g, p, l);
-  }
+    const dim3 grid(std::min(64, (n + 1023) / 1024), 1, B);
+    if (bytes) hipLaunchKernelGGL(k_fill<true>, grid, dim3(1024), 0, s, g, p, l);
+    else hipLaunchKernelGGL(k_fill<false>, grid, dim3(1024), 0, s, g, p, l);
+  }
+}
+
+void launch_expand_edges(const PyrGeom& g, const FramePlanes& p, int B, hipStream_t s) {
+  hipLaunchKernelGGL(k_expand_edges, dim3((g.total_pix / 4 + 255) / 256, B), dim3(256), 0, s, g, p);
 }
 
 void launch_tile_points(const PyrGeom& g, const FramePlanes& p, int B, hipStream_t s, int which) {
```

Measured after the change: 112,900. -1.3%, worse.
